# vLAR-group/OGC

Measured on AMD Instinct MI355X. Metric: point-clouds/sec (8192 pts) segnet fwd+bwd, higher is better.
Workload: dtype f32; 1 GPU; C4 KITTI-SF train_seg unsup: segnet_kitti fwd + OGC loss (dynamic+smooth+invariance) + bwd + Adam, 4 samples x 4 views x 8192 pts per GPU; n_point=8192, n_slot=10, parallelism=dp1, optimizer_stepped=True

## Files before the change

include/ogc_ops.h:

```cpp
#ifndef OGC_OPS_H
#define OGC_OPS_H

#ifdef __cplusplus
extern "C" {
#endif

typedef void *ogc_stream_t;
typedef unsigned short ogc_bf16_t;

enum {
    OGC_OK = 0,
    OGC_ERR_INVALID_ARG = -1,
    OGC_ERR_LAUNCH = -2,
    OGC_ERR_UNSUPPORTED = -3
};

#define OGC_VERSION 205
int ogc_version(void);
int ogc_distance_contracted(void);
int ogc_set_deterministic(int on);
int ogc_get_deterministic(void);
const char *ogc_last_error(void);

int ogc_furthest_point_sampling(int b, int n, int m, const float *xyz, float *temp,
                                int *idx, ogc_stream_t stream);

int ogc_furthest_point_sampling_chain(int b, int n, int m, const float *xyz, float *temp, int *idx,
                                      const int *ties_in, int *ties_out, ogc_stream_t stream);

int ogc_gather_points(int b, int c, int n, int npoints, const float *points, const int *idx,
                      float *out, ogc_stream_t stream);

int ogc_gather_points_grad(int b, int c, int n, int npoints, const float *grad_out,
                           const int *idx, float *grad_points, ogc_stream_t stream);

int ogc_knn(int b, int n, int m, int k, const float *unknown, const float *known,
            float *dist2, int *idx, ogc_stream_t stream);

int ogc_three_nn(int b, int n, int m, const float *unknown, const float *known, float *dist2,
                 int *idx, ogc_stream_t stream);

int ogc_three_interpolate(int b, int c, int m, int n, const float *points, const int *idx,
                          const float *weight, float *out, ogc_stream_t stream);

int ogc_three_interpolate_grad(int b, int c, int n, int m, const float *grad_out,
                               const int *idx, const float *weight, float *grad_points,
                               ogc_stream_t stream);

int ogc_group_points(int b, int c, int n, int npoints, int nsample, const float *points,
                     const int *idx, float *out, ogc_stream_t stream);

int ogc_group_points_grad(int b, int c, int n, int npoints, int nsample, const float *grad_out,
                          const int *idx, float *grad_points, ogc_stream_t stream);

int ogc_ball_query(int b, int n, int m, float radius, int nsample, const float *new_xyz,
                   const float *xyz, int *idx, ogc_stream_t stream);


int ogc_knn_clamped(int b, int n, int m, int k, float radius, const float *unknown,
                    const float *known, float *dist, int *idx, ogc_stream_t stream);

long long ogc_cell_grid_bytes(int b, int n);
int ogc_cell_grid_build(int b, int n, float radius, const float *xyz, void *grid, ogc_stream_t stream);
int ogc_ball_query_cells(int b, int n, float radius, int nsample, const float *xyz, const void *grid, float grid_radius, int *idx,
                         ogc_stream_t stream);
int ogc_knn_clamped_cells(int b, int n, int k, float radius, const float *xyz, void *grid, float grid_radius, float *dist, int *idx,
                          ogc_stream_t stream);

int ogc_adam_max_tensors(void);
int ogc_adam_chunk(void);
int ogc_adam_step(int n_tensors, int n_chunks, const long long *table, const int *chunks, const void *const *grad_ptrs,
                  float *step_snapshot, int *flag, double lr, double beta1, double beta2, double eps, double weight_decay,
                  ogc_stream_t stream);

int ogc_kabsch_rotation(int nb, const float *S, float *R, int *valid, ogc_stream_t stream);

int ogc_group_concat(int b, int c, int n, int npoints, int nsample, const float *xyz, const float *new_xyz,
                     const float *points, const int *idx, float *out, ogc_stream_t stream);

int ogc_group_concat_grad(int b, int c, int n, int npoints, int nsample, const float *grad_out, const int *idx,
                          float *grad_points, ogc_stream_t stream);

int ogc_group_linear_fwd(int b, int m, int n, int npoints, int nsample, int groups, const float *P, const int *idx,
                         const float *rel, const float *wx, float *y, double *stats, ogc_stream_t stream);
int ogc_group_linear_fwd_direct(int b, int m, int cf, int n, int npoints, int nsample, int groups, const float *feats,
                                const int *idx, const float *rel, const float *w, float *y, double *stats, ogc_stream_t stream);
int ogc_group_linear_fwd_direct_h(int b, int m, int cf, int n, int npoints, int nsample, int groups, const float *feats,
                                  const int *idx, const float *rel, const float *w, ogc_bf16_t *y, double *stats, ogc_stream_t stream);
int ogc_group_linear_bwd(int b, int m, int n, int npoints, int nsample, const float *grad_y, const int *idx,
                         const float *rel, float *grad_p, float *dwx, ogc_stream_t stream);

int ogc_group_reverse_chunk(int n, int npoints, int nsample);
int ogc_group_reverse(int b, int n, int npoints, int nsample, const int *idx, int *rev_start, unsigned short *rev_pos,
                      unsigned short *heads, ogc_stream_t stream);
int ogc_group_points_grad_rev(int b, int c, int n, int npoints, int nsample, const float *grad_out, const int *rev_start,
                              const unsigned short *rev_pos, const unsigned short *heads, float *grad_points,
                              ogc_stream_t stream);

int ogc_group_points_grad_rev_dwx(int b, int c, int n, int npoints, int nsample, const float *grad_out, const int *rev_start,
                                  const unsigned short *rev_pos, const unsigned short *heads, const float *rel,
// ... 73 lines not shown

int ogc_mlp_chain_pool_supported(int c0, int c1, int c2, int c3, int nsample);
int ogc_mlp_chain_pool(int b, int c0, int c1, int c2, int c3, int p, int nsample, const float *x, const float *wt1,
                       const float *b1, const float *wt2, const float *b2, const float *wt3, const float *b3, float *out,
                       ogc_stream_t stream);

int ogc_corr_layer_pool_supported(int cf, int c1, int c2, int c3, int nsample);
int ogc_corr_layer_pool(int b, int cf, int c1, int c2, int c3, int n1, int n2, int nsample, const float *pos1,
                        const float *pos2, const float *feat1, const float *feat2, const int *idx, const float *wt1,
                        const float *b1, const float *wt2, const float *b2, const float *wt3, const float *b3, float *out,
                        ogc_stream_t stream);

long long ogc_slot_masks_ws_floats(int b, int d, int n, int k);
int ogc_slot_masks_fwd(int b, int d, int n, int k, float temperature, const float *feats, const float *slots,
                       float *mask, ogc_stream_t stream);
int ogc_slot_masks_bwd(int b, int d, int n, int k, float temperature, const float *feats, const float *slots,
                       const float *mask, const float *grad_mask, float *grad_feats, float *grad_slots, float *ws,
                       ogc_stream_t stream);

int ogc_group_norm_stats_slots(void);
int ogc_group_norm_bwd_slots(void);
int ogc_group_norm_fwd(int b, int c, int hw, int groups, float eps, int relu, const float *x,
                       const float *gamma, const float *beta, float *y, float *mean, float *rstd,
                       double *ws, ogc_stream_t stream);
int ogc_group_norm_bwd(int b, int c, int hw, int groups, int relu, const float *x, const float *gamma,
                       const float *beta, const float *mean, const float *rstd, const float *grad_y,
                       float *grad_x, float *grad_gamma, float *grad_beta, double *ws, ogc_stream_t stream);

int ogc_group_norm_maxpool_fwd(int b, int c, int p, int s, int groups, float eps, int relu, const float *x,
                               const float *gamma, const float *beta, float *out, int *argmax, float *mean,
                               float *rstd, double *ws, ogc_stream_t stream);
int ogc_group_norm_maxpool_bwd(int b, int c, int p, int s, int groups, int relu, const float *x,
                               const float *gamma, const float *mean, const float *rstd, const float *out,
                               const int *argmax, const float *grad_out, float *grad_x, float *grad_gamma,
                               float *grad_beta, double *ws, ogc_stream_t stream);
int ogc_group_norm_maxpool_bwd_ext(int b, int c, int p, int s, int groups, int relu, const float *x,
                                   const float *x_at_argmax, const float *gamma, const float *mean, const float *rstd,
                                   const float *out, const int *argmax, const float *grad_out, float *grad_x,
                                   float *grad_gamma, float *grad_beta, double *ws, ogc_stream_t stream);

int ogc_batch_norm_fwd(int b, int c, int hw, float eps, int relu, int training, float momentum, const float *x,
                       const float *gamma, const float *beta, float *running_mean, float *running_var, float *y,
                       float *mean, float *rstd, double *ws, const double *stats, int slots, ogc_stream_t stream);
int ogc_batch_norm_bwd(int b, int c, int hw, int relu, int training, const float *x, const float *gamma,
                       const float *beta, const float *mean, const float *rstd, const float *grad_y, float *grad_x,
                       float *grad_gamma, float *grad_beta, double *ws, ogc_stream_t stream);
int ogc_batch_norm_maxpool_fwd(int b, int c, int p, int s, float eps, int relu, int training, float momentum,
                               const float *x, const float *gamma, const float *beta, float *running_mean,
                               float *running_var, float *out, int *argmax, float *mean, float *rstd, double *ws,
                               const double *stats, int slots, ogc_stream_t stream);
int ogc_batch_norm_maxpool_bwd(int b, int c, int p, int s, int relu, int training, const float *x, const float *gamma,
                               const float *mean, const float *rstd, const float *out, const int *argmax,
                               const float *grad_out, float *grad_x, float *grad_gamma, float *grad_beta, double *ws,
                               ogc_stream_t stream);

int ogc_conv1x1_wgrad(int b, int cin, int cout, int hw, const float *x, const float *dy, float *dw,
                      ogc_stream_t stream);

int ogc_conv1x1_gemm(int b, int M, int K, int hw, int transpose_a, const float *w, const float *in,
                     float *out, ogc_stream_t stream);

int ogc_conv1x1_gn_slots(void);
int ogc_conv1x1_gemm_stats_supported(int b, int M, int K, int hw, int affine);
int ogc_conv1x1_gemm_stream_supported(int b, int M, int K, int hw);
int ogc_conv1x1_gemm_any(int b, int M, int K, int hw, int transpose_a, const float *w, const float *in, float *out,
                         ogc_stream_t stream);

int ogc_set_matmul_precision(int bf16);
int ogc_conv1x1_gemm_gnstats(int b, int M, int K, int hw, int groups, const float *w, const float *in, float *out,
                             double *stats, ogc_stream_t stream);

int ogc_group_norm_coeffs(int b, int c, int hw, int groups, float eps, const float *x, const float *gamma,
                          const float *beta, const double *stats, int slots, double *ws, float *mean, float *rstd,
                          float *a, float *bb, ogc_stream_t stream);
int ogc_conv1x1_gemm_affine(int b, int M, int K, int hw, int relu, int groups, const float *w, const float *in,
                            const float *pa, const float *pb, float *out, double *stats, ogc_stream_t stream);
int ogc_conv1x1_wgrad_affine(int b, int cin, int cout, int hw, int relu, const float *x, const float *pa,
                             const float *pb, const float *dy, float *dw, ogc_stream_t stream);
int ogc_conv1x1_wgrad_affine_pooled(int b, int cin, int cout, int hw, int relu, int nsample, const float *x, const float *pa,
                                    const float *pb, const float *y, const float *coef2, const float *inj, float *dw,
                                    ogc_stream_t stream);
int ogc_conv1x1_dgrad_pooled(int b, int cin, int cout, int hw, int nsample, const float *w, const float *y, const float *coef2,
                             const float *inj, float *grad_z, ogc_stream_t stream);

int ogc_group_norm_fwd_stats(int b, int c, int hw, int groups, float eps, int relu, const float *x,
                             const float *gamma, const float *beta, float *y, float *mean, float *rstd,
                             const double *stats, int slots, ogc_stream_t stream);
int ogc_group_norm_maxpool_fwd_stats(int b, int c, int p, int s, int groups, float eps, int relu, const float *x,
                                     const float *gamma, const float *beta, float *out, int *argmax, float *mean,
                                     float *rstd, const double *stats, int slots, ogc_stream_t stream);

int ogc_conv1x1_gemm_affine_pool(int b, int M, int K, int hw, int relu, int groups, int nsample, const float *w,
                                 const float *in, const float *pa, const float *pb, const float *next_gamma,
                                 float *out, double *stats, float *yext, int *aext, ogc_stream_t stream);
int ogc_group_norm_pool_extremes(int b, int c, int p, int s, int groups, float eps, int relu, const float *yext,
                                 const int *aext, const float *gamma, const float *beta, float *out, int *argmax,
                                 float *mean, float *rstd, const double *stats, int slots, ogc_stream_t stream);

int ogc_chamfer_terms(int b, int n1, int n2, int p, const float *p1, const float *pc2, const int *idx12, const int *idx21,
                      float *dist1, float *dist2, ogc_stream_t stream);
int ogc_chamfer_terms_grad(int b, int n1, int n2, int p, const float *p1, const float *pc2, const int *idx12, const int *idx21,
                           const float *g1, const float *g2, float *grad_p1, ogc_stream_t stream);

int ogc_gather_xyz_pair(int b, int n, int m, const float *xyz, const int *idx, float *out, float *out_t, ogc_stream_t stream);
int ogc_flow_advance(int b, int n, float scale, const float *cur, const float *delta, const float *ref, float *out_delta,
                     float *out_new, float *out_new_t, float *out_flow, ogc_stream_t stream);
int ogc_linear_cn(int b, int cin, int cout, int n, const float *x, const float *weight, const float *bias, float *y,
                  ogc_stream_t stream);
int ogc_three_nn_weights(int b, int n, int mode, const float *dist2, float *weight, ogc_stream_t stream);
int ogc_soft_corr_flow(int b, int n1, int n2, int c, float support, const float *epsilon, const float *pc1, const float *pc2,
                       const float *f1, const float *f2, float *flow, ogc_stream_t stream);
int ogc_gru_reset(int b, int c, int cx, int n, int s, const float *rc, long long rc_batch_stride, const float *hx, float *out,
                  ogc_stream_t stream);
int ogc_gru_blend(int b, int c, int n, int s, const float *zc, long long zc_batch_stride, const float *qc,
                  long long qc_batch_stride, const float *h, long long h_batch_stride, float *out, ogc_stream_t stream);

int ogc_zero_arena_begin(void *base, int bytes, ogc_stream_t stream);
int ogc_zero_arena_end(void);

int ogc_group_linear_fwd_h(int b, int m, int n, int npoints, int nsample, int groups, const float *P, const int *idx,
                           const float *rel, const float *wx, ogc_bf16_t *y, double *stats, ogc_stream_t stream);
int ogc_group_linear_fwd_pt_h(int b, int m, int n, int npoints, int nsample, int groups, const float *Pt, const int *idx,
                              const float *rel, const float *wx, ogc_bf16_t *y, double *stats, ogc_stream_t stream);
int ogc_group_points_grad_rev_h(int b, int c, int n, int npoints, int nsample, const ogc_bf16_t *grad_out, const int *rev_start,
                                const unsigned short *rev_pos, const unsigned short *heads, float *grad_points,
                                ogc_stream_t stream);
int ogc_group_points_grad_rev_dwx_h(int b, int c, int n, int npoints, int nsample, const ogc_bf16_t *grad_out, const int *rev_start,
                                    const unsigned short *rev_pos, const unsigned short *heads, const float *rel,
                                    float *grad_points, float *dwx, ogc_stream_t stream);
int ogc_conv1x1_gemm_h(int b, int M, int K, int hw, int transpose_a, const float *w, const ogc_bf16_t *in, ogc_bf16_t *out,
                       ogc_stream_t stream);
int ogc_conv1x1_gemm_affine_h(int b, int M, int K, int hw, int relu, int groups, const float *w, const ogc_bf16_t *in,
                              const float *pa, const float *pb, ogc_bf16_t *out, double *stats, ogc_stream_t stream);
int ogc_conv1x1_gemm_affine_pool_h(int b, int M, int K, int hw, int relu, int groups, int nsample, const float *w,
                                   const ogc_bf16_t *in, const float *pa, const float *pb, const float *next_gamma,
                                   ogc_bf16_t *out, double *stats, float *yext, int *aext, ogc_stream_t stream);
int ogc_conv1x1_wgrad_xf_h(int b, int cin, int cout, int hw, const float *x, const ogc_bf16_t *dy, float *dw,
                           ogc_stream_t stream);
int ogc_conv1x1_wgrad_affine_h(int b, int cin, int cout, int hw, int relu, const ogc_bf16_t *x, const float *pa,
                               const float *pb, const ogc_bf16_t *dy, float *dw, ogc_stream_t stream);
int ogc_conv1x1_wgrad_affine_pooled_h(int b, int cin, int cout, int hw, int relu, int nsample, const ogc_bf16_t *x,
                                      const float *pa, const float *pb, const ogc_bf16_t *y, const float *coef2,
                                      const float *inj, float *dw, ogc_stream_t stream);
int ogc_conv1x1_dgrad_pooled_h(int b, int cin, int cout, int hw, int nsample, const float *w, const ogc_bf16_t *y,
                               const float *coef2, const float *inj, ogc_bf16_t *grad_z, ogc_stream_t stream);
int ogc_conv1x1_wgrad_moments_h(int b, int cin, int cout, int hw, int relu, const ogc_bf16_t *y_prev, const float *pa,
                                const float *pb, const ogc_bf16_t *grad_y, float *moments, ogc_stream_t stream);
int ogc_conv1x1_wgrad_moments_pooled_h(int b, int cin, int cout, int hw, int relu, int nsample, const ogc_bf16_t *y_prev,
                                       const float *pa, const float *pb, const ogc_bf16_t *y, const float *coef2,
                                       const float *inj, float *moments, ogc_stream_t stream);
int ogc_conv1x1_dgrad_adjoint_h(int b, int cin, int cout, int hw, int relu, const float *w, const ogc_bf16_t *grad_y,
                                const ogc_bf16_t *y_prev, const float *pa, const float *pb, const float *coef,
                                ogc_bf16_t *grad_prev, ogc_stream_t stream);
int ogc_conv1x1_dgrad_adjoint_pooled_h(int b, int cin, int cout, int hw, int relu, int nsample, const float *w,
                                       const ogc_bf16_t *y, const float *coef2, const float *inj, const ogc_bf16_t *y_prev,
                                       const float *pa, const float *pb, const float *coef, ogc_bf16_t *grad_prev,
                                       ogc_stream_t stream);
int ogc_group_norm_bwd_h(int b, int c, int hw, int groups, int relu, const ogc_bf16_t *x, const float *gamma,
                         const float *beta, const float *mean, const float *rstd, const ogc_bf16_t *grad_y,
                         ogc_bf16_t *grad_x, float *grad_gamma, float *grad_beta, double *ws, ogc_stream_t stream);
int ogc_group_norm_maxpool_bwd_sparse_h(int b, int c, int p, int s, int groups, int relu, const ogc_bf16_t *x,
                                        const float *x_at_argmax, const float *gamma, const float *mean, const float *rstd,
                                        const float *out, const int *argmax, const float *grad_out, float *coef2, float *inj,
                                        float *grad_gamma, float *grad_beta, double *ws, ogc_stream_t stream);

#ifdef __cplusplus
// ... 4 lines not shown
```

ogc_amd/_lib.py:

```python
import ctypes
import os

_HERE = os.path.dirname(os.path.abspath(__file__))
FMAD = os.environ.get("OGC_FMAD", "0") == "1"
DETERMINISTIC = os.environ.get("OGC_DETERMINISTIC", "0") == "1"
LIB_PATH = os.path.join(_HERE, "csrc", "libogc_ops_fmad.so" if FMAD else "libogc_ops.so")

_vp = ctypes.c_void_p
_int = ctypes.c_int
_flt = ctypes.c_float
_dbl = ctypes.c_double
_ll = ctypes.c_longlong

SIGNATURES = {
    "ogc_set_deterministic": [_int],
    "ogc_group_linear_fwd_direct": [_int, _int, _int, _int, _int, _int, _int, _vp, _vp, _vp, _vp, _vp, _vp, _vp],
    "ogc_get_deterministic": [],
    "ogc_furthest_point_sampling": [_int, _int, _int, _vp, _vp, _vp, _vp],
    "ogc_furthest_point_sampling_chain": [_int, _int, _int, _vp, _vp, _vp, _vp, _vp, _vp],
    "ogc_gather_points": [_int, _int, _int, _int, _vp, _vp, _vp, _vp],
    "ogc_gather_points_grad": [_int, _int, _int, _int, _vp, _vp, _vp, _vp],
    "ogc_knn": [_int, _int, _int, _int, _vp, _vp, _vp, _vp, _vp],
    "ogc_three_nn": [_int, _int, _int, _vp, _vp, _vp, _vp, _vp],
    "ogc_three_interpolate": [_int, _int, _int, _int, _vp, _vp, _vp, _vp, _vp],
# ... 7 lines not shown
    "ogc_view_means_grad": [_int, _vp, _vp, _vp, _vp, _vp, _vp],
    "ogc_sum_ranges": [_int, _vp, _vp, _vp, _ll, _vp, _vp],
    "ogc_three_interpolate_grad_rev_bs": [_int, _int, _int, _int, _vp, _ll, _vp, _vp, _vp, _vp, _vp, _vp],
    "ogc_group_points_grad_rev": [_int, _int, _int, _int, _int, _vp, _vp, _vp, _vp, _vp, _vp],
    "ogc_group_points_grad_rev_dwx": [_int, _int, _int, _int, _int, _vp, _vp, _vp, _vp, _vp, _vp, _vp, _vp],
    "ogc_ball_query": [_int, _int, _int, _flt, _int, _vp, _vp, _vp, _vp],
    "ogc_knn_clamped": [_int, _int, _int, _int, _flt, _vp, _vp, _vp, _vp, _vp],
    "ogc_cell_grid_bytes": [_int, _int],
    "ogc_cell_grid_build": [_int, _int, _flt, _vp, _vp, _vp],
    "ogc_ball_query_cells": [_int, _int, _flt, _int, _vp, _vp, _flt, _vp, _vp],
    "ogc_knn_clamped_cells": [_int, _int, _int, _flt, _vp, _vp, _flt, _vp, _vp, _vp],
    "ogc_chamfer_terms": [_int, _int, _int, _int, _vp, _vp, _vp, _vp, _vp, _vp, _vp],
    "ogc_chamfer_terms_grad": [_int, _int, _int, _int, _vp, _vp, _vp, _vp, _vp, _vp, _vp, _vp],
    "ogc_gather_xyz_pair": [_int, _int, _int, _vp, _vp, _vp, _vp, _vp],
    "ogc_flow_advance": [_int, _int, _flt, _vp, _vp, _vp, _vp, _vp, _vp, _vp, _vp],
    "ogc_linear_cn": [_int, _int, _int, _int, _vp, _vp, _vp, _vp, _vp],
    "ogc_three_nn_weights": [_int, _int, _int, _vp, _vp, _vp],
    "ogc_soft_corr_flow": [_int, _int, _int, _int, _flt, _vp, _vp, _vp, _vp, _vp, _vp, _vp],
    "ogc_gru_reset": [_int, _int, _int, _int, _int, _vp, _ll, _vp, _vp, _vp],
    "ogc_gru_blend": [_int, _int, _int, _int, _vp, _ll, _vp, _ll, _vp, _ll, _vp, _vp],
    "ogc_zero_arena_begin": [_vp, _int, _vp],
    "ogc_zero_arena_end": [],
    "ogc_adam_max_tensors": [],
    "ogc_adam_chunk": [],
    "ogc_adam_step": [_int, _int, _vp, _vp, _vp, _vp, _vp, _dbl, _dbl, _dbl, _dbl, _dbl, _vp],
    "ogc_kabsch_rotation": [_int, _vp, _vp, _vp, _vp],
    "ogc_lsap_maximize": [_int, _int, _vp, _vp, _vp],
    "ogc_rigid_moments": [_int, _int, _int, _vp, _vp, _vp, _vp, _vp, _vp, _vp],
    "ogc_rigid_translation": [_int, _vp, _vp, _vp, _vp, _vp],
    "ogc_rigid_blend": [_int, _int, _int, _int, _int, _vp, _vp, _vp, _vp, _vp, _vp, _vp, _vp],
    "ogc_mask_iou": [_int, _int, _int, _vp, _vp, _vp, _vp, _vp],
    "ogc_matched_distance": [_int, _int, _int, _int, _int, _vp, _vp, _vp, _vp, _vp, _vp, _vp, _vp, _vp],
    "ogc_soft_nn_target": [_int, _int, _int, _int, _flt, _vp, _vp, _vp, _vp, _vp, _vp],
    "ogc_group_concat": [_int, _int, _int, _int, _int, _vp, _vp, _vp, _vp, _vp, _vp],
    "ogc_group_linear_fwd": [_int, _int, _int, _int, _int, _int, _vp, _vp, _vp, _vp, _vp, _vp, _vp],
    "ogc_group_linear_bwd": [_int, _int, _int, _int, _int, _vp, _vp, _vp, _vp, _vp, _vp],
    "ogc_group_concat_grad": [_int, _int, _int, _int, _int, _vp, _vp, _vp, _vp],
    "ogc_neighbour_consistency_fwd": [_int, _int, _int, _int, _int, _vp, _vp, _vp, _vp],
    "ogc_reverse_neighbours": [_int, _int, _int, _vp, _vp, _vp, _vp, _vp, _vp],
    "ogc_neighbour_consistency_bwd": [_int, _int, _int, _int, _int, _vp, _vp, _vp, _vp, _vp, _vp, _vp, _vp],
    "ogc_sym_eigvals": [_int, _int, _vp, _vp, _vp],
    "ogc_group_norm_fwd": [_int, _int, _int, _int, _flt, _int, _vp, _vp, _vp, _vp, _vp, _vp, _vp, _vp],
    "ogc_group_norm_bwd": [_int, _int, _int, _int, _int, _vp, _vp, _vp, _vp, _vp, _vp, _vp, _vp, _vp, _vp, _vp],
    "ogc_group_norm_maxpool_fwd": [_int, _int, _int, _int, _int, _flt, _int, _vp, _vp, _vp, _vp, _vp, _vp, _vp, _vp, _vp],
    "ogc_conv1x1_gemm": [_int, _int, _int, _int, _int, _vp, _vp, _vp, _vp],
    "ogc_attention_fwd": [_int, _int, _int, _int, _int, _flt, _vp, _int, _vp, _int, _vp, _int, _vp, _vp, _vp],
    "ogc_attention_bwd": [_int, _int, _int, _int, _int, _flt, _vp, _int, _vp, _int, _vp, _int, _vp, _vp, _vp, _vp, _int,
                          _vp, _int, _vp, _int, _vp],
    "ogc_conv1x1_gemm_affine_pool": [_int, _int, _int, _int, _int, _int, _int, _vp, _vp, _vp, _vp, _vp, _vp, _vp, _vp, _vp,
                                     _vp],
    "ogc_group_norm_pool_extremes": [_int, _int, _int, _int, _int, _flt, _int, _vp, _vp, _vp, _vp, _vp, _vp, _vp, _vp, _vp,
                                     _int, _vp],
    "ogc_small_linear_fwd": [_int, _int, _int, _vp, _vp, _vp, _vp, _vp],
    "ogc_small_linear_bwd": [_int, _int, _int, _vp, _vp, _vp, _vp, _vp, _vp, _vp],
    "ogc_conv1x1_wgrad_moments": [_int, _int, _int, _int, _int, _vp, _vp, _vp, _vp, _vp, _vp],
    "ogc_gn_moments_combine": [_int, _int, _int, _int, _int, _vp, _vp, _vp, _vp, _vp, _vp, _vp, _vp, _vp, _vp, _vp, _vp],
    "ogc_conv1x1_dgrad_adjoint": [_int, _int, _int, _int, _int, _vp, _vp, _vp, _vp, _vp, _vp, _vp, _vp],
    "ogc_group_norm_maxpool_bwd_sparse": [_int, _int, _int, _int, _int, _int, _vp, _vp, _vp, _vp, _vp, _vp, _vp, _vp, _vp, _vp,
                                          _vp, _vp, _vp, _vp],
    "ogc_group_norm_maxpool_bwd_ext": [_int, _int, _int, _int, _int, _int, _vp, _vp, _vp, _vp, _vp, _vp, _vp, _vp, _vp, _vp,
                                       _vp, _vp, _vp],
    "ogc_conv1x1_wgrad_moments_pooled": [_int, _int, _int, _int, _int, _int, _vp, _vp, _vp, _vp, _vp, _vp, _vp, _vp],
    "ogc_conv1x1_dgrad_adjoint_pooled": [_int, _int, _int, _int, _int, _int, _vp, _vp, _vp, _vp, _vp, _vp, _vp, _vp, _vp, _vp],
    "ogc_mlp_chain_pool_supported": [_int, _int, _int, _int, _int],
    "ogc_mlp_chain_pool": [_int, _int, _int, _int, _int, _int, _int, _vp, _vp, _vp, _vp, _vp, _vp, _vp, _vp, _vp],
    "ogc_corr_layer_pool_supported": [_int, _int, _int, _int, _int],
    "ogc_corr_layer_pool": [_int, _int, _int, _int, _int, _int, _int, _int, _vp, _vp, _vp, _vp, _vp, _vp, _vp, _vp, _vp, _vp,
                            _vp, _vp, _vp],
    "ogc_slot_masks_ws_floats": [_int, _int, _int, _int],
    "ogc_slot_masks_fwd": [_int, _int, _int, _int, _flt, _vp, _vp, _vp, _vp],
    "ogc_slot_masks_bwd": [_int, _int, _int, _int, _flt, _vp, _vp, _vp, _vp, _vp, _vp, _vp, _vp],
    "ogc_conv1x1_gn_slots": [],
    "ogc_conv1x1_gemm_stats_supported": [_int, _int, _int, _int, _int],
    "ogc_conv1x1_gemm_stream_supported": [_int, _int, _int, _int],
    "ogc_conv1x1_gemm_any": [_int, _int, _int, _int, _int, _vp, _vp, _vp, _vp],
    "ogc_set_matmul_precision": [_int],
    "ogc_group_norm_stats_slots": [],
    "ogc_group_norm_bwd_slots": [],
    "ogc_group_norm_coeffs": [_int, _int, _int, _int, _flt, _vp, _vp, _vp, _vp, _int, _vp, _vp, _vp, _vp, _vp, _vp],
    "ogc_conv1x1_gemm_affine": [_int, _int, _int, _int, _int, _int, _vp, _vp, _vp, _vp, _vp, _vp, _vp],
    "ogc_conv1x1_wgrad_affine": [_int, _int, _int, _int, _int, _vp, _vp, _vp, _vp, _vp, _vp],
    "ogc_conv1x1_wgrad_affine_pooled": [_int, _int, _int, _int, _int, _int, _vp, _vp, _vp, _vp, _vp, _vp, _vp, _vp],
    "ogc_conv1x1_dgrad_pooled": [_int, _int, _int, _int, _int, _vp, _vp, _vp, _vp, _vp, _vp],
    "ogc_batch_norm_fwd": [_int, _int, _int, _flt, _int, _int, _flt, _vp, _vp, _vp, _vp, _vp, _vp, _vp, _vp, _vp, _vp,
                           _int, _vp],
    "ogc_batch_norm_bwd": [_int, _int, _int, _int, _int, _vp, _vp, _vp, _vp, _vp, _vp, _vp, _vp, _vp, _vp, _vp],
    "ogc_batch_norm_maxpool_fwd": [_int, _int, _int, _int, _flt, _int, _int, _flt, _vp, _vp, _vp, _vp, _vp, _vp, _vp,
                                   _vp, _vp, _vp, _vp, _int, _vp],
    "ogc_batch_norm_maxpool_bwd": [_int, _int, _int, _int, _int, _int, _vp, _vp, _vp, _vp, _vp, _vp, _vp, _vp, _vp,
                                   _vp, _vp, _vp],
    "ogc_conv1x1_gemm_gnstats": [_int, _int, _int, _int, _int, _vp, _vp, _vp, _vp, _vp],
    "ogc_group_norm_fwd_stats": [_int, _int, _int, _int, _flt, _int, _vp, _vp, _vp, _vp, _vp, _vp, _vp, _int, _vp],
    "ogc_group_norm_maxpool_fwd_stats": [_int, _int, _int, _int, _int, _flt, _int, _vp, _vp, _vp, _vp, _vp, _vp, _vp,
                                         _vp, _int, _vp],
    "ogc_conv1x1_wgrad": [_int, _int, _int, _int, _vp, _vp, _vp, _vp],
    "ogc_group_norm_maxpool_bwd": [_int, _int, _int, _int, _int, _int, _vp, _vp, _vp, _vp, _vp, _vp, _vp, _vp, _vp, _vp,
                                   _vp, _vp],
}

for _n in ("ogc_group_linear_fwd", "ogc_group_points_grad_rev", "ogc_conv1x1_gemm", "ogc_conv1x1_gemm_affine",
           "ogc_conv1x1_gemm_affine_pool", "ogc_conv1x1_wgrad_affine", "ogc_conv1x1_wgrad_affine_pooled",
           "ogc_conv1x1_dgrad_pooled", "ogc_conv1x1_wgrad_moments", "ogc_conv1x1_wgrad_moments_pooled",
           "ogc_conv1x1_dgrad_adjoint", "ogc_conv1x1_dgrad_adjoint_pooled", "ogc_group_norm_bwd",
           "ogc_group_norm_maxpool_bwd_sparse", "ogc_group_points_grad_rev_dwx"):
    SIGNATURES[_n + "_h"] = SIGNATURES[_n]
SIGNATURES["ogc_group_linear_fwd_direct_h"] = SIGNATURES["ogc_group_linear_fwd_direct"]
SIGNATURES["ogc_conv1x1_wgrad_xf_h"] = SIGNATURES["ogc_conv1x1_wgrad"]
SIGNATURES["ogc_group_linear_fwd_pt_h"] = SIGNATURES["ogc_group_linear_fwd"]

HEADER_VERSION = 205
_lib = None
_fns = {}


class OgcOpsError(RuntimeError):
    pass


def load():
    global _lib
    if _lib is None:
        if not os.path.exists(LIB_PATH):
            raise OgcOpsError(
                "libogc_ops.so not found at %s — build it with `python ogc_amd/csrc/build.py` "
                "(there is no CPU fallback)" % LIB_PATH)
        L = ctypes.CDLL(LIB_PATH)
        for name, argtypes in SIGNATURES.items():
            fn = getattr(L, name)
            fn.argtypes = argtypes
            fn.restype = _int
        L.ogc_version.restype = _int
        if L.ogc_version() != HEADER_VERSION:
            raise OgcOpsError("libogc_ops.so at %s is version %d, this package binds version %d of include/ogc_ops.h — rebuild it "
                              "with `python ogc_amd/csrc/build.py --force`" % (LIB_PATH, L.ogc_version(), HEADER_VERSION))
        L.ogc_distance_contracted.restype = _int
        if bool(L.ogc_distance_contracted()) != FMAD:
            raise OgcOpsError("%s evaluates distances %s, OGC_FMAD asked for the other form" %
                              (LIB_PATH, "contracted (fma)" if L.ogc_distance_contracted() else "un-contracted"))
        L.ogc_slot_masks_ws_floats.restype = ctypes.c_longlong
        L.ogc_cell_grid_bytes.restype = ctypes.c_longlong
        L.ogc_last_error.restype = ctypes.c_char_p
        L.ogc_set_deterministic(1 if DETERMINISTIC else 0)
        _lib = L
    return _lib


def set_deterministic(on):
    global DETERMINISTIC
    DETERMINISTIC = bool(on)
    load().ogc_set_deterministic(1 if on else 0)


CALL_COUNTS = None

ROCTX_NAMES = {
    "ogc_furthest_point_sampling": "K1 furthest_point_sampling", "ogc_furthest_point_sampling_chain": "K1 furthest_point_sampling (chain)",
    "ogc_gather_points": "K2 gather_points", "ogc_gather_points_grad": "K3 gather_points_grad",
    "ogc_knn": "K4 knn", "ogc_knn_clamped": "K4 knn (+ sqrt + radius clamp)", "ogc_knn_clamped_cells": "K4 knn (shared cell grid)",
    "ogc_three_nn": "K5 three_nn", "ogc_three_interpolate": "K6 three_interpolate",
    "ogc_three_interpolate_grad": "K7 three_interpolate_grad", "ogc_three_interpolate_grad_rev": "K7 three_interpolate_grad (gather form)",
    "ogc_three_interpolate_grad_rev_bs": "K7 three_interpolate_grad (gather form)",
    "ogc_group_points": "K8 group_points", "ogc_group_points_grad": "K9 group_points_grad",
    "ogc_group_points_grad_rev": "K9 group_points_grad (gather form)",
    "ogc_ball_query": "K10 ball_query", "ogc_ball_query_cells": "K10 ball_query (shared cell grid)",
}
_roctx = None


def _roctx_lib():
    global _roctx
    if _roctx is None:
        _roctx = False
        if os.environ.get("OGC_ROCTX", "0") == "1":
            for name in ("librocprofiler-sdk-roctx.so", "libroctx64.so"):
                try:
                    lib = ctypes.CDLL(os.path.join(os.environ.get("ROCM_PATH", "/opt/rocm"), "lib", name))
                    lib.roctxRangePushA.argtypes = [ctypes.c_char_p]
                    lib.roctxRangePushA.restype = ctypes.c_int
                    lib.roctxRangePop.restype = ctypes.c_int
                    _roctx = lib
                    break
                except (OSError, AttributeError):
                    continue
    return _roctx


def call(name, *args):
    if CALL_COUNTS is not None:
        CALL_COUNTS[name] += 1
    fn = _fns.get(name)
    if fn is None:
        fn = _fns[name] = getattr(load(), name)
    tx = _roctx_lib()
# ... 13 lines not shown
```

ogc_amd/csrc/conv1x1.hip:

```cpp
#include "conv1x1_shared.h"
#include "act_io.h"
#include "conv1x1_epilogue.h"

int ogc_g_matmul_bf16 = 0;


namespace {


template <bool TRANSPOSE_A, int KQ, bool STATS, bool PRO, bool BF, bool POOL = false, typename IT = float, typename OT = float>
__global__ __launch_bounds__(WG_WAVES *OGC_WAVE) void conv1x1_gemm_kernel(int M, int K, int hw, int groups,
                                                                          const float *__restrict__ w,
                                                                          const IT *__restrict__ in,
                                                                          OT *__restrict__ out,
                                                                          double *__restrict__ stats,
                                                                          const float *__restrict__ pa,
                                                                          const float *__restrict__ pb, int pro_relu,
                                                                          PoolOut pool = PoolOut()) {
    extern __shared__ __attribute__((aligned(16))) float a_lds[];
    __shared__ double s_stats[STATS ? 64 : 1];
    __shared__ __attribute__((aligned(16))) float s_sign[POOL ? 64 : 4];
    const int lane = threadIdx.x & 63, wave = threadIdx.x >> 6;
    const int j = lane & 15, kk = lane >> 4;
    const int b = blockIdx.y;
// ... 132 lines not shown
#pragma unroll
        for (int q = 0; q < KQ; ++q) {
            if (q < Kq) {
                float av[4];
#pragma unroll
                for (int a = 0; a < 4; ++a) av[a] = a_lds[(a * 16 + j) * a_ld + q * 4 + kk];
#pragma unroll
                for (int a = 0; a < 4; ++a) {
                    if (a < nblk) {
                        acc[a][0] = __builtin_amdgcn_mfma_f32_16x16x4f32(av[a], xin[q].x, acc[a][0], 0, 0, 0);
                        acc[a][1] = __builtin_amdgcn_mfma_f32_16x16x4f32(av[a], xin[q].y, acc[a][1], 0, 0, 0);
                        acc[a][2] = __builtin_amdgcn_mfma_f32_16x16x4f32(av[a], xin[q].z, acc[a][2], 0, 0, 0);
                        acc[a][3] = __builtin_amdgcn_mfma_f32_16x16x4f32(av[a], xin[q].w, acc[a][3], 0, 0, 0);
                    }
                }
            }
        }
        }
        if (live) {
            if constexpr (sizeof(OT) == 2 && (STATS || POOL)) {
#pragma unroll
                for (int a = 0; a < 4; ++a)
#pragma unroll
                    for (int c = 0; c < 4; ++c)
#pragma unroll
                        for (int r = 0; r < 4; ++r) acc[a][c][r] = ogc_as_stored<OT>(acc[a][c][r]);
            }
#pragma unroll
            for (int a = 0; a < 4; ++a)
#pragma unroll
                for (int r = 0; r < 4; ++r) {
                    const int m = m0 + a * 16 + kk * 4 + r;
                    if (m < M) {
                        const float4 o = make_float4(acc[a][0][r], acc[a][1][r], acc[a][2][r], acc[a][3][r]);
                        ogc_st4(outb + (size_t)m * hw + p0 + 4 * j, o);
                    }
                }
            if constexpr (POOL) {
                const int centres = hw / pool.s;
                const int centre = (p0 + 4 * j) / pool.s;
                const size_t o0 = ((size_t)b * M + m0 + kk * 4) * centres + centre;
                if (pool.s == 64) ogc_pool_extremes_epilogue<16>(acc, nblk, s_sign, j, kk, m0, M, centres, 64, pool.yext + o0, pool.aext + o0);
                else if (pool.s == 32) ogc_pool_extremes_epilogue<8>(acc, nblk, s_sign, j, kk, m0, M, centres, 32, pool.yext + o0, pool.aext + o0);
                else ogc_pool_extremes_epilogue<4>(acc, nblk, s_sign, j, kk, m0, M, centres, 16, pool.yext + o0, pool.aext + o0);
            }
            if (STATS) {
#pragma unroll
                for (int a = 0; a < 4; ++a) {
                    if (a < nblk) {
                        float sm = 0.f, sq = 0.f;
#pragma unroll
                        for (int r = 0; r < 4; ++r)
#pragma unroll
                            for (int c = 0; c < 4; ++c) {
                                const float v = acc[a][c][r];
                                sm += v;
                                sq += v * v;
                            }
                        sm += ogc_dpp_f32<0xB1>(sm); sq += ogc_dpp_f32<0xB1>(sq);
                        sm += ogc_dpp_f32<0x4E>(sm); sq += ogc_dpp_f32<0x4E>(sq);
                        sm += ogc_dpp_f32<0x141>(sm); sq += ogc_dpp_f32<0x141>(sq);
                        sm += ogc_dpp_f32<0x140>(sm); sq += ogc_dpp_f32<0x140>(sq);
                        const int m = m0 + a * 16 + kk * 4;
                        if (j == 0 && m < M) {
                            const int g = m / cpg;
                            atomicAdd(&s_stats[2 * g], (double)sm);
                            atomicAdd(&s_stats[2 * g + 1], (double)sq);
                        }
                    }
                }
            }
        }
    }
    if (STATS) {
        __syncthreads();
        if (threadIdx.x < 2 * groups) {
            const int slot = blockIdx.x % GN_SLOTS;
            double *dst = stats + ((size_t)slot * gridDim.y + b) * 2 * groups;
            atomicAdd(dst + threadIdx.x, s_stats[threadIdx.x]);
        }
    }
}

template <int KQ, bool PRO, bool EXACT, bool STATS = false, bool POOL = false, bool DUAL = false, bool TRANS = false>
__global__ __launch_bounds__(WG_WAVES *OGC_WAVE, DUAL ? 2 : 1) void conv1x1_gemm_stream_kernel(int M, int K, int hw, int ntiles,
                                                                                 const float *__restrict__ w,
                                                                                 const float *__restrict__ in,
                                                                                 float *__restrict__ out,
                                                                                 const float *__restrict__ pa,
                                                                                 const float *__restrict__ pb, int pro_relu,
                                                                                 int groups = 1, int nbatch = 1,
                                                                                 double *__restrict__ stats = nullptr,
                                                                                 PoolOut pool = PoolOut()) {
    extern __shared__ __attribute__((aligned(16))) float a_lds[];
    const int lane = threadIdx.x & 63, wave = __builtin_amdgcn_readfirstlane(threadIdx.x >> 6);
    const int j = lane & 15, kk = lane >> 4;
    const int Kq = (K + 3) >> 2, Mt = (M + 63) >> 6, a_ld = ogc_a_ld(Kq);
    const int tiles_per_img = hw >> 6;
    for (int mt = 0; mt < Mt; ++mt)
        ogc_stage_weight_tile<TRANS, WG_WAVES>(a_lds + (size_t)mt * 64 * a_ld, w, mt * 64, M, K, Kq);
    float *sgn_all = a_lds + (size_t)Mt * 64 * a_ld + (PRO ? WG_WAVES * 2 * FW_KQ_MAX * 4 : 0) + WG_WAVES * 4 * 16 * 2 * 2;
    if constexpr (POOL) {
        for (int t = threadIdx.x; t < Mt * 64; t += WG_WAVES * OGC_WAVE) sgn_all[t] = (t < M && pool.sign[t] < 0.f) ? -1.f : 1.f;
    }
    __syncthreads();
    const int nw = gridDim.x * WG_WAVES;
    const unsigned off_main = (unsigned)(kk * hw + 4 * j);
    const unsigned off_last = (unsigned)(min(kk, K - 1 - (Kq - 1) * 4) * hw + 4 * j);
    auto load_tile = [&](int t, float4(&x)[KQ]) {
        t = min(t, ntiles - 1);
        const int b = t / tiles_per_img, p0 = (t - b * tiles_per_img) * 64;
        const float *inb = in + (size_t)b * K * hw + p0;
#pragma unroll
        for (int q = 0; q < KQ; ++q)
            if (EXACT || q < Kq) {
                const float *rowq = inb + (size_t)(q * 4) * hw;
                x[q] = *reinterpret_cast<const float4 *>(rowq + ((EXACT ? q == KQ - 1 : q == Kq - 1) ? off_last : off_main));
            }
    };
    float *cw = a_lds + (size_t)Mt * 64 * a_ld + wave * (2 * KQ * 4);
    int coef_b = -1;
    double *sacc = reinterpret_cast<double *>(a_lds + (size_t)Mt * 64 * a_ld + (PRO ? WG_WAVES * 2 * FW_KQ_MAX * 4 : 0)) +
                   wave * (4 * 16 * 2);
    int stat_b = -1;
    auto flush_stats = [&]() {
        if constexpr (STATS) {
            if (stat_b >= 0) {
                const int cpg = M / groups;
                double *dst = stats + ((size_t)(blockIdx.x % GN_SLOTS) * nbatch + stat_b) * 2 * groups;
                if (lane < Mt * 16) {
                    const int m = (lane >> 4) * 64 + ((lane >> 2) & 3) * 16 + (lane & 3) * 4;
                    if (m < M) {
                        unsafeAtomicAdd(dst + 2 * (m / cpg), sacc[2 * lane]);
                        unsafeAtomicAdd(dst + 2 * (m / cpg) + 1, sacc[2 * lane + 1]);
                    }
                }
            }
            if (lane < 64) { sacc[2 * lane] = 0.0; sacc[2 * lane + 1] = 0.0; }
            __builtin_amdgcn_wave_barrier();
        }
    };
    auto compute_store = [&](int t, float4(&x)[KQ]) {
        const int b = t / tiles_per_img, p0 = (t - b * tiles_per_img) * 64;
        if constexpr (STATS) {
            if (b != stat_b) { flush_stats(); stat_b = b; }
        }
        if (PRO) {
            if (b != coef_b) {
                coef_b = b;
                for (int r = lane; r < KQ * 4; r += OGC_WAVE) {
                    cw[r] = r < K ? pa[(size_t)b * K + r] : 0.f;
                    cw[KQ * 4 + r] = r < K ? pb[(size_t)b * K + r] : 0.f;
                }
                __builtin_amdgcn_wave_barrier();
            }
#pragma unroll
            for (int q = 0; q < KQ; ++q) {
                if (EXACT || q < Kq) {
                    const float ca = cw[q * 4 + kk], cb = cw[KQ * 4 + q * 4 + kk];
                    float4 v = x[q];
                    v.x = fmaf(ca, v.x, cb); v.y = fmaf(ca, v.y, cb);
                    v.z = fmaf(ca, v.z, cb); v.w = fmaf(ca, v.w, cb);
                    if (pro_relu) { v.x = fmaxf(v.x, 0.f); v.y = fmaxf(v.y, 0.f); v.z = fmaxf(v.z, 0.f); v.w = fmaxf(v.w, 0.f); }
                    x[q] = v;
                }
            }
        }
        float *outb = out + (size_t)b * M * hw + p0;
        const unsigned off_out = (unsigned)(kk * 4 * hw + 4 * j);
        for (int mt = 0; mt < Mt; ++mt) {
            const float *at = a_lds + (size_t)mt * 64 * a_ld;
            const int nblk = EXACT ? 4 : min(4, (M - mt * 64 + 15) >> 4);
            v4f acc[4][4];
#pragma unroll
            for (int a = 0; a < 4; ++a)
#pragma unroll
                for (int c = 0; c < 4; ++c) acc[a][c] = (v4f){0.f, 0.f, 0.f, 0.f};
#pragma unroll
            for (int q = 0; q < KQ; ++q) {
                if (EXACT || q < Kq) {
                    float av[4];
#pragma unroll
                    for (int a = 0; a < 4; ++a) av[a] = at[(a * 16 + j) * a_ld + q * 4 + kk];
#pragma unroll
                    for (int a = 0; a < 4; ++a) {
                        if (EXACT || a < nblk) {
                            acc[a][0] = __builtin_amdgcn_mfma_f32_16x16x4f32(av[a], x[q].x, acc[a][0], 0, 0, 0);
                            acc[a][1] = __builtin_amdgcn_mfma_f32_16x16x4f32(av[a], x[q].y, acc[a][1], 0, 0, 0);
                            acc[a][2] = __builtin_amdgcn_mfma_f32_16x16x4f32(av[a], x[q].z, acc[a][2], 0, 0, 0);
                            acc[a][3] = __builtin_amdgcn_mfma_f32_16x16x4f32(av[a], x[q].w, acc[a][3], 0, 0, 0);
                        }
                    }
                }
            }
#pragma unroll
            for (int a = 0; a < 4; ++a)
#pragma unroll
                for (int r = 0; r < 4; ++r) {
                    const int m0 = mt * 64 + a * 16 + r;
                    if (EXACT || m0 + kk * 4 < M)
                        *reinterpret_cast<float4 *>(outb + (size_t)m0 * hw + off_out) =
                            make_float4(acc[a][0][r], acc[a][1][r], acc[a][2][r], acc[a][3][r]);
                }
            if constexpr (POOL) {
                const int m0p = mt * 64;
                const int centres = hw / pool.s;
                const int centre = (p0 + 4 * j) / pool.s;
                const size_t o0 = ((size_t)b * M + m0p + kk * 4) * centres + centre;
                const float *sg = sgn_all + m0p;
                if (pool.s == 64) ogc_pool_extremes_epilogue<16>(acc, nblk, sg, j, kk, m0p, M, centres, 64, pool.yext + o0, pool.aext + o0);
                else if (pool.s == 32) ogc_pool_extremes_epilogue<8>(acc, nblk, sg, j, kk, m0p, M, centres, 32, pool.yext + o0, pool.aext + o0);
                else ogc_pool_extremes_epilogue<4>(acc, nblk, sg, j, kk, m0p, M, centres, 16, pool.yext + o0, pool.aext + o0);
            }
            if constexpr (STATS) {
#pragma unroll
                for (int a = 0; a < 4; ++a) {
                    if (EXACT || a < nblk) {
                        float sm = 0.f, sq = 0.f;
#pragma unroll
                        for (int r = 0; r < 4; ++r)
#pragma unroll
                            for (int c = 0; c < 4; ++c) {
                                const float v = acc[a][c][r];
                                sm += v;
                                sq += v * v;
                            }
                        sm += ogc_dpp_f32<0xB1>(sm); sq += ogc_dpp_f32<0xB1>(sq);
                        sm += ogc_dpp_f32<0x4E>(sm); sq += ogc_dpp_f32<0x4E>(sq);
                        sm += ogc_dpp_f32<0x141>(sm); sq += ogc_dpp_f32<0x141>(sq);
                        sm += ogc_dpp_f32<0x140>(sm); sq += ogc_dpp_f32<0x140>(sq);
                        if (j == 0) {
                            const int slot = (mt * 4 + a) * 4 + kk;
                            sacc[2 * slot] += (double)sm;
                            sacc[2 * slot + 1] += (double)sq;
                        }
                    }
                }
            }
        }
    };
    const int per = (ntiles + nw - 1) / nw;
    int t = (blockIdx.x * WG_WAVES + wave) * per;
    const int t_end = min(ntiles, t + per);
    if (STATS) flush_stats();
    if constexpr (DUAL) {
        float4 x1[KQ];
        for (; t < t_end; ++t) {
            load_tile(t, x1);
            compute_store(t, x1);
        }
        if (STATS) flush_stats();
        return;
    }
    float4 xa[KQ], xb[KQ];
    if (t < t_end) {
        load_tile(t, xa);
        for (; t + 1 < t_end; t += 2) {
            load_tile(t + 1, xb);
            compute_store(t, xa);
            load_tile(t + 2, xa);
            compute_store(t + 1, xb);
        }
        if (t < t_end) compute_store(t, xa);
    }
    if (STATS) flush_stats();
}

bool gemm_stream_eligible(int b, int M, int K, int hw, bool pro, bool pool = false, bool any_precision = false) {
    const int Kq = (K + 3) / 4, Mt = (M + 63) / 64;
    const long long ntiles = (long long)b * (hw / 64);
    const size_t lds = ((size_t)Mt * 64 * ogc_a_ld(Kq) + (pro ? WG_WAVES * 2 * FW_KQ_MAX * 4 : 0)) * sizeof(float) +
                       WG_WAVES * 4 * 16 * 2 * sizeof(double) + (pool ? (size_t)Mt * 64 * sizeof(float) : 0);
    static const bool off = getenv("OGC_GEMM_STREAM") && getenv("OGC_GEMM_STREAM")[0] == '0';
    return !(off || (g_matmul_bf16 && !any_precision) || (hw & 63) != 0 || Kq <= 25 || Kq > FW_KQ_MAX || lds > 156 * 1024 || ntiles < 2048 ||
             ntiles >= (1ll << 31));
}

template <bool PRO, bool STATS = false, bool POOL = false, bool TRANS = false>
bool gemm_stream_launch(int b, int M, int K, int hw, const float *w, const float *in, float *out, const float *pa,
                        const float *pb, int pro_relu, hipStream_t s, int groups = 1, double *stats = nullptr,
                        PoolOut pool = PoolOut()) {
    const int Kq = (K + 3) / 4, Mt = (M + 63) / 64;
    const long long ntiles = (long long)b * (hw / 64);
    const size_t lds = ((size_t)Mt * 64 * ogc_a_ld(Kq) + (PRO ? WG_WAVES * 2 * FW_KQ_MAX * 4 : 0)) * sizeof(float) +
                       WG_WAVES * 4 * 16 * 2 * sizeof(double) + (POOL ? (size_t)Mt * 64 * sizeof(float) : 0);
    if (!gemm_stream_eligible(b, M, K, hw, PRO, POOL, STATS) || lds > 156 * 1024) return false;
    const int wgs = (int)(ntiles / WG_WAVES < 256 ? ntiles / WG_WAVES : 256);
#define OGC_STREAM_D(KQV, EX, DU, WGS)                                                                                       \
    do {                                                                                                                     \
        static bool raised = false;                                                                                          \
        const void *fn = reinterpret_cast<const void *>(&conv1x1_gemm_stream_kernel<KQV, PRO, EX, STATS, POOL, DU, TRANS>);         \
        if (!raised) {                                                                                                       \
            if (hipFuncSetAttribute(fn, hipFuncAttributeMaxDynamicSharedMemorySize, 156 * 1024) != hipSuccess) return false;  \
            raised = true;                                                                                                   \
        }                                                                                                                    \
        hipLaunchKernelGGL((conv1x1_gemm_stream_kernel<KQV, PRO, EX, STATS, POOL, DU, TRANS>), dim3(WGS), dim3(WG_WAVES * OGC_WAVE), \
                           lds, s, M, K, hw, (int)ntiles, w, in, out, pa, pb, pro_relu, groups, b, stats, pool);             \
    } while (0)
    static const bool dual_on = !(getenv("OGC_GEMM_STREAM_DUAL") && getenv("OGC_GEMM_STREAM_DUAL")[0] == '0');
    const bool dual = dual_on && !POOL && 2 * (lds + 1024) <= 156 * 1024 && ntiles >= 4096;
    const int wgs2 = (int)(ntiles / WG_WAVES < 512 ? ntiles / WG_WAVES : 512);
#define OGC_STREAM(KQV, EX)                                                                                                  \
    do {                                                                                                                     \
        if (dual) OGC_STREAM_D(KQV, EX, true, wgs2);                                                                         \
        else OGC_STREAM_D(KQV, EX, false, wgs);                                                                              \
    } while (0)
    const bool full_rows = M % 64 == 0;
    if (Kq == 32 && full_rows) OGC_STREAM(32, true);
    else if (Kq == 33 && full_rows) OGC_STREAM(33, true);
    else if (Kq <= 33) OGC_STREAM(33, false);
    else OGC_STREAM(40, false);
#undef OGC_STREAM
#undef OGC_STREAM_D
    return true;
}

template <bool T, bool STATS, bool PRO, bool POOL = false, typename AT = float>
int gemm_launch(int b, int M, int K, int hw, int groups, const float *w, const AT *in, AT *out, double *stats,
                const float *pa, const float *pb, int pro_relu, hipStream_t s, PoolOut pool = PoolOut()) {
    const int Kq = (K + 3) / 4;
    constexpr bool F32 = sizeof(AT) == 4;
    if constexpr (F32 && !T && (!POOL || (STATS && PRO))) {
        static const bool wide_fp32 = [] { const char *e = getenv("OGC_BF16_WIDE_STATS"); return e && e[0] == '1'; }();
        if ((!g_matmul_bf16 || (STATS && wide_fp32)) &&
            gemm_stream_launch<PRO, STATS, POOL>(b, M, K, hw, w, in, out, pa, pb, pro_relu, s, groups, stats, pool))
            return OGC_OK;
    }
    if constexpr (F32 && T && !STATS && !PRO && !POOL) {
        if (!g_matmul_bf16 && gemm_stream_launch<false, false, false, true>(b, M, K, hw, w, in, out, pa, pb, pro_relu, s))
            return OGC_OK;
    }
    if constexpr (F32) {
        if (!g_matmul_bf16 && ogc_gemm32_launch(T, STATS, PRO, POOL, b, M, K, hw, groups, w, in, out, stats, pa, pb, pro_relu, s,
                                                pool.sign, pool.yext, pool.aext, pool.s))
            return OGC_OK;
    }
    if constexpr (!F32) {
        if (ogc_gemm16_launch(T, STATS, PRO, POOL, b, M, K, hw, groups, w, in, out, stats, pa, pb, pro_relu, s, pool.sign, pool.yext,
                              pool.aext, pool.s))
            return OGC_OK;
    }
    const size_t lds = (size_t)64 * ogc_a_ld(Kq) * sizeof(float);
    dim3 grid(ogc_divup(hw, 64 * WG_WAVES), b);
#define OGC_GEMM(KQV)                                                                                                  \
    do {                                                                                                               \
        if constexpr (!F32)                                                                                            \
            hipLaunchKernelGGL((conv1x1_gemm_kernel<T, KQV, STATS, PRO, true, POOL, AT, AT>), grid,                     \
                               dim3(WG_WAVES * OGC_WAVE), lds, s, M, K, hw, groups, w, in, out, stats, pa, pb, pro_relu, pool); \
        else if (g_matmul_bf16)                                                                                        \
            hipLaunchKernelGGL((conv1x1_gemm_kernel<T, KQV, STATS, PRO, true, POOL>), grid, dim3(WG_WAVES * OGC_WAVE), \
                               lds, s, M, K, hw, groups, w, in, out, stats, pa, pb, pro_relu, pool);                   \
        else                                                                                                           \
            hipLaunchKernelGGL((conv1x1_gemm_kernel<T, KQV, STATS, PRO, false, POOL>), grid, dim3(WG_WAVES * OGC_WAVE), \
                               lds, s, M, K, hw, groups, w, in, out, stats, pa, pb, pro_relu, pool);                   \
    } while (0)
    if (Kq <= 2) OGC_GEMM(2);
    else if (Kq <= 8) OGC_GEMM(8);
    else if (Kq <= 16) OGC_GEMM(16);
    else if (Kq <= 25) OGC_GEMM(25);
    else if (POOL && !g_matmul_bf16) return OGC_ERR_UNSUPPORTED;
    else {
        if (Kq <= 33) OGC_GEMM(33);
        else OGC_GEMM(40);
    }
#undef OGC_GEMM
    return OGC_OK;
}

template <typename AT>
int gemm_check(const char *name, int b, int M, int K, int hw, const float *w, const AT *in, const AT *out) {
    OGC_REQUIRE(b >= 0 && M >= 1 && K >= 1 && hw >= 1, "%s: bad shape", name);
    OGC_REQUIRE(w && in && out, "%s: null pointer", name);
    if ((hw & 63) != 0 || K > 4 * FW_KQ_MAX || (((uintptr_t)in | (uintptr_t)out) & ogc_act_mask<AT>()) != 0) {
        ogc_set_error("%s: needs hw %% 64 == 0, K <= %d and 16-byte aligned tensors (hw=%d, K=%d)", name,
                      4 * FW_KQ_MAX, hw, K);
        return OGC_ERR_UNSUPPORTED;
    }
    if (sizeof(AT) == 2 && !g_matmul_bf16) {
        ogc_set_error("%s: 16-bit activations need ogc_set_matmul_precision(1)", name);
        return OGC_ERR_UNSUPPORTED;
    }
    OGC_REQUIRE((long long)M * hw < (1ll << 31) && (long long)K * hw < (1ll << 31) && b <= 65535,
                "%s: one sample exceeds 32-bit indexing", name);
    return OGC_OK;
}

}

namespace {
template <typename AT>
int gemm_plain_impl(const char *name, int b, int M, int K, int hw, int transpose_a, const float *w, const AT *in, AT *out,
                    ogc_stream_t stream) {
    const int rc = gemm_check(name, b, M, K, hw, w, in, out);
    if (rc != OGC_OK) return rc;
    if (b == 0) return OGC_OK;
    if (transpose_a)
        gemm_launch<true, false, false, false, AT>(b, M, K, hw, 1, w, in, out, nullptr, nullptr, nullptr, 0, (hipStream_t)stream);
    else
        gemm_launch<false, false, false, false, AT>(b, M, K, hw, 1, w, in, out, nullptr, nullptr, nullptr, 0, (hipStream_t)stream);
    OGC_CHECK_LAUNCH(name);
    return OGC_OK;
}
}

extern "C" int ogc_conv1x1_gemm(int b, int M, int K, int hw, int transpose_a, const float *w, const float *in,
                                float *out, ogc_stream_t stream) {
    return gemm_plain_impl<float>("ogc_conv1x1_gemm", b, M, K, hw, transpose_a, w, in, out, stream);
}

extern "C" int ogc_conv1x1_gemm_h(int b, int M, int K, int hw, int transpose_a, const float *w, const ogc_bf16_t *in,
                                  ogc_bf16_t *out, ogc_stream_t stream) {
    return gemm_plain_impl<ogc_bf16>("ogc_conv1x1_gemm_h", b, M, K, hw, transpose_a, w, in, out, stream);
}

extern "C" int ogc_conv1x1_gn_slots(void) { return GN_SLOTS; }

extern "C" int ogc_conv1x1_gemm_stats_supported(int b, int M, int K, int hw, int affine) {
    if (b < 1 || M < 1 || K < 1 || hw < 1) return 0;
    return (K <= 100 || g_matmul_bf16 || gemm_stream_eligible(b, M, K, hw, affine != 0, false, true)) ? 1 : 0;
}

extern "C" int ogc_conv1x1_gemm_stream_supported(int b, int M, int K, int hw) {
    if (b < 1 || M < 1 || K < 1 || hw < 1) return 0;
    return gemm_stream_eligible(b, M, K, hw, false) ? 1 : 0;
}

extern "C" int ogc_set_matmul_precision(int bf16) {
    const int previous = g_matmul_bf16;
    g_matmul_bf16 = bf16 ? 1 : 0;
    return previous;
}

extern "C" int ogc_conv1x1_gemm_gnstats(int b, int M, int K, int hw, int groups, const float *w, const float *in,
                                        float *out, double *stats, ogc_stream_t stream) {
    const int rc = gemm_check<float>("ogc_conv1x1_gemm_gnstats", b, M, K, hw, w, in, out);
    if (rc != OGC_OK) return rc;
    OGC_REQUIRE(stats, "ogc_conv1x1_gemm_gnstats: null pointer");
    if (groups < 1 || groups > 32 || M % groups != 0 || (M / groups) % 4 != 0) {
        ogc_set_error("ogc_conv1x1_gemm_gnstats: needs 1 <= groups <= 32 and (M / groups) %% 4 == 0 (M=%d, groups=%d)", M,
                      groups);
        return OGC_ERR_UNSUPPORTED;
    }
    if (K > 100 && !g_matmul_bf16 && !gemm_stream_eligible(b, M, K, hw, false, false, true)) {
        ogc_set_error("ogc_conv1x1_gemm_gnstats: not profitable for K > 100 (K=%d) on this shape; use ogc_conv1x1_gemm", K);
        return OGC_ERR_UNSUPPORTED;
    }
    if (b == 0) return OGC_OK;
    if (ogc_zero_async(stats, sizeof(double) * 2 * GN_SLOTS * (size_t)b * groups, (hipStream_t)stream) != hipSuccess) {
        ogc_set_error("ogc_conv1x1_gemm_gnstats: memset failed");
        return OGC_ERR_LAUNCH;
    }
    gemm_launch<false, true, false>(b, M, K, hw, groups, w, in, out, stats, nullptr, nullptr, 0, (hipStream_t)stream);
    OGC_CHECK_LAUNCH("ogc_conv1x1_gemm_gnstats");
    return OGC_OK;
}


namespace {
template <typename AT>
int gemm_affine_impl(const char *name, int b, int M, int K, int hw, int relu, int groups, const float *w, const AT *in,
                     const float *pa, const float *pb, AT *out, double *stats, ogc_stream_t stream) {
    const int rc = gemm_check(name, b, M, K, hw, w, in, out);
    if (rc != OGC_OK) return rc;
    OGC_REQUIRE(pa && pb, "ogc_conv1x1_gemm_affine: null pointer");
    if (b == 0) return OGC_OK;
    hipStream_t s = (hipStream_t)stream;
    if (groups > 0) {
        OGC_REQUIRE(stats, "ogc_conv1x1_gemm_affine: null pointer");
        if (groups > 32 || M % groups != 0 || (M / groups) % 4 != 0 || (K > 100 && !g_matmul_bf16 && !gemm_stream_eligible(b, M, K, hw, true, false, true))) {
            ogc_set_error("ogc_conv1x1_gemm_affine: output statistics need groups <= 32, (M / groups) %% 4 == 0, K <= 100 "
                          "(or a shape of the streaming kernel: ogc_conv1x1_gemm_stats_supported)");
            return OGC_ERR_UNSUPPORTED;
        }
        if (ogc_zero_async(stats, sizeof(double) * 2 * GN_SLOTS * (size_t)b * groups, s) != hipSuccess) {
            ogc_set_error("ogc_conv1x1_gemm_affine: memset failed");
            return OGC_ERR_LAUNCH;
        }
        gemm_launch<false, true, true, false, AT>(b, M, K, hw, groups, w, in, out, stats, pa, pb, relu, s);
    } else {
        gemm_launch<false, false, true, false, AT>(b, M, K, hw, 1, w, in, out, nullptr, pa, pb, relu, s);
    }
    OGC_CHECK_LAUNCH(name);
    return OGC_OK;
}
}

extern "C" int ogc_conv1x1_gemm_affine(int b, int M, int K, int hw, int relu, int groups, const float *w, const float *in,
                                       const float *pa, const float *pb, float *out, double *stats,
                                       ogc_stream_t stream) {
    return gemm_affine_impl<float>("ogc_conv1x1_gemm_affine", b, M, K, hw, relu, groups, w, in, pa, pb, out, stats, stream);
}

extern "C" int ogc_conv1x1_gemm_affine_h(int b, int M, int K, int hw, int relu, int groups, const float *w, const ogc_bf16_t *in,
                                         const float *pa, const float *pb, ogc_bf16_t *out, double *stats,
                                         ogc_stream_t stream) {
    return gemm_affine_impl<ogc_bf16>("ogc_conv1x1_gemm_affine_h", b, M, K, hw, relu, groups, w, in, pa, pb, out, stats, stream);
}

namespace {
template <typename AT>
int gemm_affine_pool_impl(const char *name, int b, int M, int K, int hw, int relu, int groups, int nsample, const float *w,
                          const AT *in, const float *pa, const float *pb, const float *next_gamma, AT *out, double *stats,
                          float *yext, int *aext, ogc_stream_t stream) {
    const int rc = gemm_check(name, b, M, K, hw, w, in, out);
// ... 40 lines not shown
```

ogc_amd/csrc/conv1x1_shared.h:

```cpp
#pragma once
#include <stdlib.h>

#include "ogc_common.h"
#include "conv_stage.h"

typedef float v4f __attribute__((ext_vector_type(4)));
typedef short v4s __attribute__((ext_vector_type(4)));

constexpr int WG_WAVES = 4;

extern int ogc_g_matmul_bf16;
#define g_matmul_bf16 ogc_g_matmul_bf16

__device__ __forceinline__ v4s ogc_pack_bf16(float a, float b, float c, float d) {
    typedef float v2f __attribute__((ext_vector_type(2)));
    typedef __bf16 v2bf __attribute__((ext_vector_type(2)));
    union { v2bf h[2]; v4s s; } u;
    u.h[0] = __builtin_convertvector((v2f){a, b}, v2bf);
    u.h[1] = __builtin_convertvector((v2f){c, d}, v2bf);
    return u.s;
}
```

ogc_amd/csrc/gemm_chunk.hip:

```cpp
#include <stdlib.h>

#include "ogc_common.h"
#include "act_io.h"
#include "conv1x1_shared.h"

namespace {

constexpr int GC_WAVES = 4;

__device__ __forceinline__ v4s gc_pack_bf16(float a, float b, float c, float d) { return ogc_pack_bf16_rr(a, b, c, d); }

template <int RB, int KQ, bool SPLIT_M, bool TRANS, bool POOLED = false, int KA = 1, typename AT = float, bool BF = false,
          bool TAB = false>
__global__ __launch_bounds__(GC_WAVES *OGC_WAVE, 2) void gemm_chunk_kernel(int M, int K, int hw, const float *__restrict__ w,
                                                                         const AT *__restrict__ in,
                                                                         AT *__restrict__ out,
                                                                         const float2 *__restrict__ coef2 = nullptr,
                                                                         const float2 *__restrict__ inj = nullptr,
                                                                         int s_shift = 0) {
    constexpr int KC = 4 * KQ, KCA = KC * KA, LD = 4 * ((KQ * KA) | 1);
    constexpr int MT = SPLIT_M ? 64 * RB : 16 * RB;
    constexpr int PER = (MT * KCA) / (GC_WAVES * OGC_WAVE);
    static_assert((MT * KCA) % (GC_WAVES * OGC_WAVE) == 0 && PER >= 1 && (KA == 1 || KA == 2), "staging split");
    extern __shared__ __attribute__((aligned(16))) float gc_lds[];
    const int t = threadIdx.x, lane = t & 63, wave = __builtin_amdgcn_readfirstlane(t >> 6);
    const int j = lane & 15, kk = lane >> 4;
    const int b = blockIdx.z;
    const int m0 = blockIdx.y * MT;
    const int wrow = SPLIT_M ? wave * 16 * RB : 0;
    const int p0 = SPLIT_M ? blockIdx.x * 64 : (blockIdx.x * GC_WAVES + wave) * 64;
    const bool active = p0 < hw;
    const int pl = active ? p0 : 0;
    const int nblk = min(RB, (M - m0 - wrow + 15) >> 4);
    const AT *inb = in + (size_t)b * K * hw + pl + 4 * j;
    const int nchunks = (K + KC - 1) / KC;

    v4f acc[RB][4];
#pragma unroll
    for (int a = 0; a < RB; ++a)
#pragma unroll
        for (int c = 0; c < 4; ++c) acc[a][c] = (v4f){0.f, 0.f, 0.f, 0.f};

    auto load_a = [&](int k0, float(&av)[PER]) {
#pragma unroll
        for (int i = 0; i < PER; ++i) {
            const int e = t + i * (GC_WAVES * OGC_WAVE);
            int mi, ki;
            if (TRANS) { mi = e % MT; ki = e / MT; } else { mi = e / KCA; ki = e % KCA; }
            const int m = m0 + mi, k = k0 + ki;
            const bool ok = m < M && k < K;
            const int mc = min(m, M - 1), kc = min(k, K - 1);
            const float v = TRANS ? w[(size_t)kc * M + mc] : w[(size_t)mc * K + kc];
            av[i] = ok ? v : 0.f;
        }
    };
    auto store_a = [&](float *dst, const float(&av)[PER]) {
#pragma unroll
        for (int i = 0; i < PER; ++i) {
            const int e = t + i * (GC_WAVES * OGC_WAVE);
            int mi, ki;
            if (TRANS) { mi = e % MT; ki = e / MT; } else { mi = e / KCA; ki = e % KCA; }
            dst[mi * LD + ki] = av[i];
        }
    };
    constexpr int NP = (POOLED && !TAB) ? KQ : 1;
    const int centres = hw >> s_shift;
    const int my_centre = (pl + 4 * j) >> s_shift, jpos = (pl + 4 * j) & ((1 << s_shift) - 1);
    const int cpw = 64 >> s_shift;
    float4 *tab = reinterpret_cast<float4 *>(gc_lds + 2 * MT * LD) + (size_t)wave * K * cpw;
    if constexpr (POOLED && TAB) {
        for (int e = lane; e < K * cpw; e += OGC_WAVE) {
            const int row = e / cpw, centre = (pl >> s_shift) + (e - row * cpw);
            const float2 c2v = coef2[(size_t)b * K + row];
            const float2 jj = centre < centres ? inj[((size_t)b * K + row) * centres + centre] : make_float2(0.f, __int_as_float(-1));
            tab[e] = make_float4(c2v.x, c2v.y, jj.x, jj.y);
        }
        __builtin_amdgcn_wave_barrier();
    }
    const int mine_c = (4 * j) >> s_shift;
    auto load_in = [&](int k0, float4(&xv)[KQ], float2(&cc)[NP], float2(&jv)[NP]) {
#pragma unroll
        for (int q = 0; q < KQ; ++q) {
            const int k = min(k0 + 4 * q + kk, K - 1);
            xv[q] = ogc_ld4(inb + (size_t)k * hw);
            if constexpr (POOLED && !TAB) {
                cc[q] = coef2[(size_t)b * K + k];
                jv[q] = inj[((size_t)b * K + k) * centres + my_centre];
            }
        }
    };
    auto rebuild = [&](int k0, float4(&xv)[KQ], const float2(&cc)[NP], const float2(&jv)[NP]) {
        if constexpr (POOLED && TAB) {
#pragma unroll
            for (int q = 0; q < KQ; ++q) {
                const float4 te = tab[min(k0 + 4 * q + kk, K - 1) * cpw + mine_c];
                const int rel = __float_as_int(te.w) - jpos;
                xv[q].x = fmaf(te.x, xv[q].x, te.y) + (rel == 0 ? te.z : 0.f);
                xv[q].y = fmaf(te.x, xv[q].y, te.y) + (rel == 1 ? te.z : 0.f);
                xv[q].z = fmaf(te.x, xv[q].z, te.y) + (rel == 2 ? te.z : 0.f);
                xv[q].w = fmaf(te.x, xv[q].w, te.y) + (rel == 3 ? te.z : 0.f);
            }
        } else if constexpr (POOLED) {
#pragma unroll
            for (int q = 0; q < KQ; ++q) {
                const int rel = __float_as_int(jv[q].y) - jpos;
                const float ag = jv[q].x;
                xv[q].x = fmaf(cc[q].x, xv[q].x, cc[q].y) + (rel == 0 ? ag : 0.f);
                xv[q].y = fmaf(cc[q].x, xv[q].y, cc[q].y) + (rel == 1 ? ag : 0.f);
                xv[q].z = fmaf(cc[q].x, xv[q].z, cc[q].y) + (rel == 2 ? ag : 0.f);
                xv[q].w = fmaf(cc[q].x, xv[q].w, cc[q].y) + (rel == 3 ? ag : 0.f);
            }
        }
        if (k0 + KC > K) {
#pragma unroll
            for (int q = 0; q < KQ; ++q)
                if (k0 + 4 * q + kk >= K) xv[q] = make_float4(0.f, 0.f, 0.f, 0.f);
        }
    };
    auto compute = [&](const float *a_lds, const float4(&xv)[KQ], int koff = 0) {
        if constexpr (BF) {
            static_assert(!BF || KQ % 4 == 0, "bf16 operands: whole groups of four row quads per input chunk");
#pragma unroll
            for (int g = 0; g < KQ / 4; ++g) {
                const float4 v0 = xv[4 * g], v1 = xv[4 * g + 1], v2 = xv[4 * g + 2], v3 = xv[4 * g + 3];
                const v4s bx = gc_pack_bf16(v0.x, v1.x, v2.x, v3.x);
                const v4s by = gc_pack_bf16(v0.y, v1.y, v2.y, v3.y);
                const v4s bz = gc_pack_bf16(v0.z, v1.z, v2.z, v3.z);
                const v4s bw = gc_pack_bf16(v0.w, v1.w, v2.w, v3.w);
                const float *ar = a_lds + (wrow + j) * LD + koff + 16 * g + kk;
#pragma unroll
                for (int a = 0; a < RB; ++a) {
                    const v4s av = gc_pack_bf16(ar[a * 16 * LD], ar[a * 16 * LD + 4], ar[a * 16 * LD + 8], ar[a * 16 * LD + 12]);
                    acc[a][0] = __builtin_amdgcn_mfma_f32_16x16x16bf16_1k(av, bx, acc[a][0], 0, 0, 0);
                    acc[a][1] = __builtin_amdgcn_mfma_f32_16x16x16bf16_1k(av, by, acc[a][1], 0, 0, 0);
                    acc[a][2] = __builtin_amdgcn_mfma_f32_16x16x16bf16_1k(av, bz, acc[a][2], 0, 0, 0);
                    acc[a][3] = __builtin_amdgcn_mfma_f32_16x16x16bf16_1k(av, bw, acc[a][3], 0, 0, 0);
                }
            }
        } else {
#pragma unroll
            for (int q = 0; q < KQ; ++q) {
                const float bx = xv[q].x, by = xv[q].y, bz = xv[q].z, bw = xv[q].w;
#pragma unroll
                for (int a = 0; a < RB; ++a) {
                    const float av = a_lds[(wrow + a * 16 + j) * LD + koff + q * 4 + kk];
                    acc[a][0] = __builtin_amdgcn_mfma_f32_16x16x4f32(av, bx, acc[a][0], 0, 0, 0);
                    acc[a][1] = __builtin_amdgcn_mfma_f32_16x16x4f32(av, by, acc[a][1], 0, 0, 0);
                    acc[a][2] = __builtin_amdgcn_mfma_f32_16x16x4f32(av, bz, acc[a][2], 0, 0, 0);
                    acc[a][3] = __builtin_amdgcn_mfma_f32_16x16x4f32(av, bw, acc[a][3], 0, 0, 0);
                }
            }
        }
    };

    float *buf0 = gc_lds, *buf1 = gc_lds + MT * LD;
    float4 x0[KQ], x1[KQ];
    float2 c0[NP], c1[NP], j0[NP], j1[NP];
    float a_next[PER];
    load_a(0, a_next);
    load_in(0, x0, c0, j0);
    store_a(buf0, a_next);
    __syncthreads();
    const bool work = nblk > 0;
    if constexpr (KA == 2) {
        const int npairs = (nchunks + 1) / 2;
        for (int p = 0; p < npairs; ++p) {
            const bool more = p + 1 < npairs;
            if (more) load_a((p + 1) * KCA, a_next);
            load_in((2 * p + 1) * KC, x1, c1, j1);
            rebuild(2 * p * KC, x0, c0, j0);
            if (work) compute(buf0, x0, 0);
            if (more) load_in((2 * p + 2) * KC, x0, c0, j0);
            rebuild((2 * p + 1) * KC, x1, c1, j1);
            if (work) compute(buf0, x1, KC);
            if (more) store_a(buf1, a_next);
            __syncthreads();
            float *tmp = buf0; buf0 = buf1; buf1 = tmp;
        }
    } else
    for (int i = 0; i < nchunks; i += 2) {
        const bool more1 = i + 1 < nchunks, more2 = i + 2 < nchunks;
        if (more1) {
            load_a((i + 1) * KC, a_next);
            load_in((i + 1) * KC, x1, c1, j1);
        }
        rebuild(i * KC, x0, c0, j0);
        if (work) compute(buf0, x0);
        if (more1) store_a(buf1, a_next);
        __syncthreads();
        if (!more1) break;
        if (more2) {
            load_a((i + 2) * KC, a_next);
            load_in((i + 2) * KC, x0, c0, j0);
        }
        rebuild((i + 1) * KC, x1, c1, j1);
        if (work) compute(buf1, x1);
        if (more2) store_a(buf0, a_next);
        __syncthreads();
    }
    if (!active) return;
    AT *ob = out + (size_t)b * M * hw + p0 + 4 * j;
#pragma unroll
    for (int a = 0; a < RB; ++a) {
        if (a < nblk) {
#pragma unroll
            for (int r = 0; r < 4; ++r) {
                const int m = m0 + wrow + a * 16 + kk * 4 + r;
                if (m < M) ogc_st4(ob + (size_t)m * hw, make_float4(acc[a][0][r], acc[a][1][r], acc[a][2][r], acc[a][3][r]));
            }
        }
    }
}

template <int RB, int KQ, bool SPLIT_M, int KA = 1>
void gemm_chunk_launch(int b, int M, int K, int hw, int transpose_a, const float *w, const float *in, float *out,
                       hipStream_t s) {
    constexpr int MT = SPLIT_M ? 64 * RB : 16 * RB;
    const size_t lds = (size_t)2 * MT * 4 * ((KQ * KA) | 1) * sizeof(float);
    dim3 grid(SPLIT_M ? hw / 64 : ogc_divup(hw, 64 * GC_WAVES), ogc_divup(M, MT), b);
#define GC_GO(TR, BFV)                                                                                                           \
    hipLaunchKernelGGL((gemm_chunk_kernel<RB, KQ, SPLIT_M, TR, false, KA, float, BFV>), grid, dim3(GC_WAVES * OGC_WAVE), lds, s, M, K, \
                       hw, w, in, out, nullptr, nullptr, 0)
    if (ogc_g_matmul_bf16) {
        if (transpose_a) GC_GO(true, true);
        else GC_GO(false, true);
    } else {
        if (transpose_a) GC_GO(true, false);
        else GC_GO(false, false);
    }
#undef GC_GO
}

}

extern "C" int ogc_conv1x1_gemm_any(int b, int M, int K, int hw, int transpose_a, const float *w, const float *in, float *out,
                                    ogc_stream_t stream) {
    OGC_REQUIRE(b >= 0 && M >= 1 && K >= 1 && hw >= 1, "ogc_conv1x1_gemm_any: bad shape");
    OGC_REQUIRE(w && in && out, "ogc_conv1x1_gemm_any: null pointer");
    if ((hw & 63) != 0 || (((uintptr_t)in | (uintptr_t)out) & 15) != 0) {
        ogc_set_error("ogc_conv1x1_gemm_any: needs hw %% 64 == 0 and 16-byte aligned tensors (hw=%d)", hw);
        return OGC_ERR_UNSUPPORTED;
    }
    OGC_REQUIRE((long long)M * hw < (1ll << 31) && (long long)K * hw < (1ll << 31) && b <= 65535,
                "ogc_conv1x1_gemm_any: one sample exceeds 32-bit indexing");
    if (b == 0) return OGC_OK;
    hipStream_t s = (hipStream_t)stream;
    const long long tiles = (long long)b * (hw / 64);
#define GC_CASE(RBV, KQV, SPLIT)                                                              \
    case RBV: gemm_chunk_launch<RBV, KQV, SPLIT>(b, M, K, hw, transpose_a, w, in, out, s); break
    if (tiles >= 4096) {
        const int ntile = ogc_divup(M, 128), rb = ogc_divup(M, 16 * ntile);
        switch (rb) {
            GC_CASE(1, 8, false); GC_CASE(2, 8, false); GC_CASE(3, 8, false); GC_CASE(4, 8, false);
            GC_CASE(5, 8, false); GC_CASE(6, 8, false); GC_CASE(7, 4, false);
            default: {
                static const char *kq = getenv("OGC_GEMM_CHUNK_KQ");
                if (kq && kq[0] == '4') gemm_chunk_launch<8, 4, false>(b, M, K, hw, transpose_a, w, in, out, s);
                else gemm_chunk_launch<8, 4, false, 2>(b, M, K, hw, transpose_a, w, in, out, s);
            }
        }
    } else {
        const bool same_rows = 128 * ogc_divup(M, 128) == 64 * ogc_divup(M, 64);
        const int rb = (M > 64 && same_rows && tiles * ogc_divup(M, 128) >= 512) ? 2 : 1;
        switch (rb) {
            GC_CASE(2, 8, true);
            default: gemm_chunk_launch<1, 8, true>(b, M, K, hw, transpose_a, w, in, out, s);
        }
    }
#undef GC_CASE
    OGC_CHECK_LAUNCH("ogc_conv1x1_gemm_any");
    return OGC_OK;
}

namespace {
template <typename AT>
int dgrad_pooled_impl(int b, int cin, int cout, int hw, int nsample, const float *w, const AT *y, const float *coef2,
                      const float *inj, AT *grad_z, ogc_stream_t stream) {
    constexpr bool BF = sizeof(AT) == 2;
    OGC_REQUIRE(b >= 0 && cin >= 1 && cout >= 1 && hw >= 1, "ogc_conv1x1_dgrad_pooled: bad shape");
    OGC_REQUIRE(w && y && coef2 && inj && grad_z, "ogc_conv1x1_dgrad_pooled: null pointer");
    const int sh = nsample == 16 ? 4 : nsample == 32 ? 5 : nsample == 64 ? 6 : -1;
    if (sh < 0 || hw % nsample != 0 || (hw & 63) != 0 || (long long)b * (hw / 64) < 1024 ||
        (((uintptr_t)y | (uintptr_t)grad_z) & ogc_act_mask<AT>()) != 0 || (((uintptr_t)coef2 | (uintptr_t)inj) & 7) != 0 ||
        (BF && !ogc_g_matmul_bf16)) {
        ogc_set_error("ogc_conv1x1_dgrad_pooled: needs nsample in {16, 32, 64} dividing hw, hw %% 64 == 0, >= 1024 tiles of 64 "
                      "positions and aligned tensors (hw=%d, nsample=%d, b=%d)", hw, nsample, b);
        return OGC_ERR_UNSUPPORTED;
    }
    OGC_REQUIRE((long long)cin * hw < (1ll << 31) && (long long)cout * hw < (1ll << 31) && b <= 65535,
                "ogc_conv1x1_dgrad_pooled: one sample exceeds 32-bit indexing");
    if (b == 0) return OGC_OK;
    hipStream_t s = (hipStream_t)stream;
    const float2 *c2 = reinterpret_cast<const float2 *>(coef2), *ij = reinterpret_cast<const float2 *>(inj);
    const int M = cin, K = cout;
    static const bool tab_off = [] { const char *e = getenv("OGC_DGRAD_POOLED_TAB"); return e && e[0] == '0'; }();
    const size_t tab_bytes = (size_t)GC_WAVES * K * (64 >> sh) * sizeof(float4);
    const bool tab = !tab_off && tab_bytes <= 24 * 1024;
    if (M <= 64) {
        constexpr int RB = 4, KQ = 4, KA = 2;
        dim3 grid(ogc_divup(hw, 64 * GC_WAVES), ogc_divup(M, 16 * RB), b);
        const size_t lds = (size_t)2 * 16 * RB * 4 * ((KQ * KA) | 1) * sizeof(float);
        if (tab)
            hipLaunchKernelGGL((gemm_chunk_kernel<RB, KQ, false, true, true, KA, AT, BF, true>), grid, dim3(GC_WAVES * OGC_WAVE),
                               lds + tab_bytes, s, M, K, hw, w, y, grad_z, c2, ij, sh);
        else
            hipLaunchKernelGGL((gemm_chunk_kernel<RB, KQ, false, true, true, KA, AT, BF>), grid, dim3(GC_WAVES * OGC_WAVE), lds, s, M,
                               K, hw, w, y, grad_z, c2, ij, sh);
    } else {
        constexpr int RB = 8, KQ = 4;
        dim3 grid(ogc_divup(hw, 64 * GC_WAVES), ogc_divup(M, 16 * RB), b);
        const size_t lds = (size_t)2 * 16 * RB * 4 * (KQ | 1) * sizeof(float);
        if (tab)
            hipLaunchKernelGGL((gemm_chunk_kernel<RB, KQ, false, true, true, 1, AT, BF, true>), grid, dim3(GC_WAVES * OGC_WAVE),
                               lds + tab_bytes, s, M, K, hw, w, y, grad_z, c2, ij, sh);
        else
            hipLaunchKernelGGL((gemm_chunk_kernel<RB, KQ, false, true, true, 1, AT, BF>), grid, dim3(GC_WAVES * OGC_WAVE), lds, s, M, K,
                               hw, w, y, grad_z, c2, ij, sh);
    }
    OGC_CHECK_LAUNCH("ogc_conv1x1_dgrad_pooled");
    return OGC_OK;
}
}

extern "C" int ogc_conv1x1_dgrad_pooled(int b, int cin, int cout, int hw, int nsample, const float *w, const float *y,
                                        const float *coef2, const float *inj, float *grad_z, ogc_stream_t stream) {
    return dgrad_pooled_impl<float>(b, cin, cout, hw, nsample, w, y, coef2, inj, grad_z, stream);
}

extern "C" int ogc_conv1x1_dgrad_pooled_h(int b, int cin, int cout, int hw, int nsample, const float *w, const ogc_bf16_t *y,
                                          const float *coef2, const float *inj, ogc_bf16_t *grad_z, ogc_stream_t stream) {
    return dgrad_pooled_impl<ogc_bf16>(b, cin, cout, hw, nsample, w, y, coef2, inj, grad_z, stream);
}
```

ogc_amd/csrc/group_norm.hip:

```cpp
#include "ogc_common.h"
#include "act_io.h"

namespace {

constexpr int GN_THREADS = 256;

__device__ __forceinline__ void gn_block_sum2(double &a, double &b, double *smem ) {
#pragma unroll
    for (int off = 32; off > 0; off >>= 1) {
        a += __shfl_down(a, off, 64);
        b += __shfl_down(b, off, 64);
    }
    const int lane = threadIdx.x & 63, wave = threadIdx.x >> 6;
    if (lane == 0) {
        smem[wave * 2] = a;
        smem[wave * 2 + 1] = b;
    }
    __syncthreads();
    if (threadIdx.x == 0) {
        a = 0.0;
        b = 0.0;
        for (int w = 0; w < GN_THREADS / 64; ++w) {
            a += smem[w * 2];
            b += smem[w * 2 + 1];
// ... 490 lines not shown
    const float a = rstd * gamma[ch];
    a_out[t] = a;
    bb_out[t] = beta[ch] - mean * a;
}
}

extern "C" int ogc_group_norm_coeffs(int b, int c, int hw, int groups, float eps, const float *x, const float *gamma,
                                     const float *beta, const double *stats, int slots, double *ws, float *mean,
                                     float *rstd, float *a, float *bb, ogc_stream_t stream) {
    OGC_REQUIRE(b >= 0 && c >= 1 && hw >= 1 && groups >= 1 && c % groups == 0, "ogc_group_norm_coeffs: bad shape");
    if (b == 0) return OGC_OK;
    OGC_REQUIRE(gamma && beta && mean && rstd && a && bb && (stats || (ws && x)), "ogc_group_norm_coeffs: null pointer");
    hipStream_t s = (hipStream_t)stream;
    if (!stats) {
        const int rows = b * groups;
        const long long row_len = (long long)(c / groups) * hw;
        slots = launch_gn_stats(rows, row_len, x, ws, s);
        stats = ws;
    }
    hipLaunchKernelGGL(gn_coeffs_kernel, dim3(ogc_divup(b * c, 256)), dim3(256), 0, s, b, c, hw, groups, eps, gamma, beta,
                       stats, slots, mean, rstd, a, bb);
    OGC_CHECK_LAUNCH("ogc_group_norm_coeffs");
    return OGC_OK;
}

extern "C" int ogc_group_norm_stats_slots(void) { return GN_STATS_SLOTS; }
extern "C" int ogc_group_norm_bwd_slots(void) { return GN_BWD_SLOTS; }

extern "C" int ogc_group_norm_fwd(int b, int c, int hw, int groups, float eps, int relu, const float *x,
                                  const float *gamma, const float *beta, float *y, float *mean, float *rstd,
                                  double *ws, ogc_stream_t stream) {
    return gn_fwd_impl("ogc_group_norm_fwd", b, c, hw, groups, eps, relu, x, gamma, beta, y, mean, rstd, ws, nullptr, 0,
                       stream);
}

extern "C" int ogc_group_norm_fwd_stats(int b, int c, int hw, int groups, float eps, int relu, const float *x,
                                        const float *gamma, const float *beta, float *y, float *mean, float *rstd,
                                        const double *stats, int slots, ogc_stream_t stream) {
    OGC_REQUIRE(stats && slots >= 1, "ogc_group_norm_fwd_stats: no statistics");
    return gn_fwd_impl("ogc_group_norm_fwd_stats", b, c, hw, groups, eps, relu, x, gamma, beta, y, mean, rstd, nullptr,
                       stats, slots, stream);
}

namespace {
template <typename AT>
int gn_bwd_impl(int b, int c, int hw, int groups, int relu, const AT *x, const float *gamma, const float *beta, const float *mean,
                const float *rstd, const AT *grad_y, AT *grad_x, float *grad_gamma, float *grad_beta, double *ws,
                ogc_stream_t stream) {
    OGC_REQUIRE(b >= 0 && c >= 1 && hw >= 1 && groups >= 1 && c % groups == 0, "ogc_group_norm_bwd: bad shape");
    if (b == 0) return OGC_OK;
    if (sizeof(AT) == 2 && ((hw & 3) != 0 || (((uintptr_t)x | (uintptr_t)grad_y | (uintptr_t)grad_x) & 7) != 0)) {
        ogc_set_error("ogc_group_norm_bwd_h: needs hw %% 4 == 0 and 8-byte aligned tensors");
        return OGC_ERR_UNSUPPORTED;
    }
    OGC_REQUIRE(x && gamma && beta && mean && rstd && grad_y && grad_x && grad_gamma && grad_beta && ws,
                "ogc_group_norm_bwd: null pointer");
    hipStream_t s = (hipStream_t)stream;
    double *dsdb = ws;
    dim3 grid(hw_chunks(b, c, hw), c, b);
    const int slots = (int)grid.x;
    if (relu) {
        hipLaunchKernelGGL((gn_bwd_sums_kernel<true, AT>), grid, dim3(GN_THREADS), 0, s, c, hw, groups, x, gamma, beta, mean,
                           rstd, grad_y, dsdb);
        hipLaunchKernelGGL((gn_bwd_dx_kernel<true, AT>), grid, dim3(GN_THREADS), 0, s, c, hw, groups, x, gamma, beta, mean,
                           rstd, dsdb, slots, grad_y, grad_x, grad_gamma, grad_beta);
    } else {
        hipLaunchKernelGGL((gn_bwd_sums_kernel<false, AT>), grid, dim3(GN_THREADS), 0, s, c, hw, groups, x, gamma, beta, mean,
                           rstd, grad_y, dsdb);
        hipLaunchKernelGGL((gn_bwd_dx_kernel<false, AT>), grid, dim3(GN_THREADS), 0, s, c, hw, groups, x, gamma, beta, mean,
                           rstd, dsdb, slots, grad_y, grad_x, grad_gamma, grad_beta);
    }
    OGC_CHECK_LAUNCH("ogc_group_norm_bwd");
    return OGC_OK;
}
}

extern "C" int ogc_group_norm_bwd(int b, int c, int hw, int groups, int relu, const float *x, const float *gamma,
                                  const float *beta, const float *mean, const float *rstd, const float *grad_y,
                                  float *grad_x, float *grad_gamma, float *grad_beta, double *ws,
                                  ogc_stream_t stream) {
    return gn_bwd_impl<float>(b, c, hw, groups, relu, x, gamma, beta, mean, rstd, grad_y, grad_x, grad_gamma, grad_beta, ws, stream);
}

extern "C" int ogc_group_norm_bwd_h(int b, int c, int hw, int groups, int relu, const ogc_bf16_t *x, const float *gamma,
                                    const float *beta, const float *mean, const float *rstd, const ogc_bf16_t *grad_y,
                                    ogc_bf16_t *grad_x, float *grad_gamma, float *grad_beta, double *ws,
                                    ogc_stream_t stream) {
    return gn_bwd_impl<ogc_bf16>(b, c, hw, groups, relu, x, gamma, beta, mean, rstd, grad_y, grad_x, grad_gamma, grad_beta, ws, stream);
}

static bool gn_pool_shape_ok(int s) { return s >= 4 && s <= 256 && (s & (s - 1)) == 0; }

namespace {
int gn_pool_fwd_impl(const char *name, int b, int c, int p, int s, int groups, float eps, int relu, const float *x,
                     const float *gamma, const float *beta, float *out, int *argmax, float *mean, float *rstd,
                     double *ws, const double *stats, int slots, ogc_stream_t stream) {
    OGC_REQUIRE(b >= 0 && c >= 1 && p >= 1 && groups >= 1 && c % groups == 0, "%s: bad shape", name);
    if (!gn_pool_shape_ok(s) || ((uintptr_t)x & 15) != 0) {
        ogc_set_error("%s: nsample=%d must be a power of two in [4,256] and x 16-byte aligned", name, s);
        return OGC_ERR_UNSUPPORTED;
    }
    if (b == 0) return OGC_OK;
    OGC_REQUIRE(x && gamma && beta && out && argmax && mean && rstd && (ws || stats), "%s: null pointer", name);
    OGC_REQUIRE((long long)c * p * s < (1ll << 31) && b <= 65535, "%s: one sample exceeds 32-bit indexing", name);
    hipStream_t st = (hipStream_t)stream;
    if (!stats) {
        const int rows = b * groups;
        const long long row_len = (long long)(c / groups) * p * s;
        slots = launch_gn_stats(rows, row_len, x, ws, st);
        stats = ws;
    }
    const int rows_per_block = GN_THREADS / (s / 4);
    int bx = ogc_divup(p, rows_per_block);
    while (bx > 1 && (long long)bx * c * b > 8192) bx = (bx + 1) / 2;
    dim3 grid(bx, c, b);
    if (relu)
        hipLaunchKernelGGL(gn_apply_maxpool_kernel<true>, grid, dim3(GN_THREADS), 0, st, c, p, s, groups, eps, x, gamma,
                           beta, stats, slots, out, argmax, mean, rstd);
    else
        hipLaunchKernelGGL(gn_apply_maxpool_kernel<false>, grid, dim3(GN_THREADS), 0, st, c, p, s, groups, eps, x,
                           gamma, beta, stats, slots, out, argmax, mean, rstd);
    OGC_CHECK_LAUNCH(name);
    return OGC_OK;
}
}

extern "C" int ogc_group_norm_maxpool_fwd(int b, int c, int p, int s, int groups, float eps, int relu, const float *x,
                                          const float *gamma, const float *beta, float *out, int *argmax,
                                          float *mean, float *rstd, double *ws, ogc_stream_t stream) {
    return gn_pool_fwd_impl("ogc_group_norm_maxpool_fwd", b, c, p, s, groups, eps, relu, x, gamma, beta, out, argmax,
                            mean, rstd, ws, nullptr, 0, stream);
}

extern "C" int ogc_group_norm_maxpool_fwd_stats(int b, int c, int p, int s, int groups, float eps, int relu,
                                                const float *x, const float *gamma, const float *beta, float *out,
                                                int *argmax, float *mean, float *rstd, const double *stats, int slots,
                                                ogc_stream_t stream) {
    OGC_REQUIRE(stats && slots >= 1, "ogc_group_norm_maxpool_fwd_stats: no statistics");
    return gn_pool_fwd_impl("ogc_group_norm_maxpool_fwd_stats", b, c, p, s, groups, eps, relu, x, gamma, beta, out,
                            argmax, mean, rstd, nullptr, stats, slots, stream);
}

extern "C" int ogc_group_norm_pool_extremes(int b, int c, int p, int s, int groups, float eps, int relu,
                                            const float *yext, const int *aext, const float *gamma, const float *beta,
                                            float *out, int *argmax, float *mean, float *rstd, const double *stats,
                                            int slots, ogc_stream_t stream) {
    OGC_REQUIRE(b >= 0 && c >= 1 && p >= 1 && s >= 1 && groups >= 1 && c % groups == 0 && slots >= 1,
                "ogc_group_norm_pool_extremes: bad shape");
    if (b == 0) return OGC_OK;
    OGC_REQUIRE(yext && aext && gamma && beta && out && argmax && mean && rstd && stats,
                "ogc_group_norm_pool_extremes: null pointer");
    OGC_REQUIRE(b <= 65535, "ogc_group_norm_pool_extremes: too many samples for one grid");
    const dim3 grid(c, b);
    hipStream_t st = (hipStream_t)stream;
    if (relu)
        hipLaunchKernelGGL(gn_pool_extremes_kernel<true>, grid, dim3(GN_THREADS), 0, st, c, p, s, groups, eps, yext, aext,
                           gamma, beta, stats, slots, out, argmax, mean, rstd);
    else
        hipLaunchKernelGGL(gn_pool_extremes_kernel<false>, grid, dim3(GN_THREADS), 0, st, c, p, s, groups, eps, yext, aext,
                           gamma, beta, stats, slots, out, argmax, mean, rstd);
    OGC_CHECK_LAUNCH("ogc_group_norm_pool_extremes");
    return OGC_OK;
}

static int gn_maxpool_bwd_impl(int b, int c, int p, int s, int groups, int relu, const float *x, const float *x_at_argmax,
                               const float *gamma, const float *mean, const float *rstd, const float *out,
// ... 110 lines not shown
```

ogc_amd/csrc/ogc_common.h:

```cpp
#pragma once
#include <hip/hip_runtime.h>
#include <stdint.h>

#include "../../include/ogc_ops.h"

#define OGC_WAVE 64

void ogc_set_error(const char *fmt, ...);
void *ogc_workspace(hipStream_t stream, size_t bytes);

#define OGC_REQUIRE(cond, ...)            \
    do {                                  \
        if (!(cond)) {                    \
            ogc_set_error(__VA_ARGS__);   \
            return OGC_ERR_INVALID_ARG;   \
        }                                 \
    } while (0)

#define OGC_CHECK_LAUNCH(name)                                                   \
    do {                                                                         \
        hipError_t e_ = hipGetLastError();                                       \
        if (e_ != hipSuccess) {                                                  \
            ogc_set_error("%s: launch failed: %s", name, hipGetErrorString(e_)); \
            return OGC_ERR_LAUNCH;                                               \
// ... 114 lines not shown
#pragma unroll
    for (int u = 0; u < 4; ++u) dy[u] = q2y - Y[u];
#pragma unroll
    for (int u = 0; u < 4; ++u) dz[u] = q2z - Z[u];
#ifdef OGC_FMAD
#pragma unroll
    for (int u = 0; u < 4; ++u) s[u] = ogc_sqsum3(dx[u], dy[u], dz[u]);
#else
#pragma unroll
    for (int u = 0; u < 4; ++u) dx[u] = dx[u] * dx[u];
#pragma unroll
    for (int u = 0; u < 4; ++u) dy[u] = dy[u] * dy[u];
#pragma unroll
    for (int u = 0; u < 4; ++u) dz[u] = dz[u] * dz[u];
#pragma unroll
    for (int u = 0; u < 4; ++u) s[u] = dx[u] + dy[u];
#pragma unroll
    for (int u = 0; u < 4; ++u) s[u] = s[u] + dz[u];
#endif
#pragma unroll
    for (int u = 0; u < 4; ++u) {
        d[2 * u] = s[u].x;
        d[2 * u + 1] = s[u].y;
    }
}

__device__ __forceinline__ void ogc_tile_fetch(const float *__restrict__ pts, int n, int t, int lane,
                                               float (&r)[8][3]) {
#pragma unroll
    for (int i = 0; i < 8; ++i) {
        const int p = t * OGC_TILE + i * OGC_WAVE + lane;
        if (p < n) {
            const float *q = pts + (size_t)p * 3;
            r[i][0] = q[0]; r[i][1] = q[1]; r[i][2] = q[2];
        } else {
            r[i][0] = r[i][1] = r[i][2] = INFINITY;
        }
    }
}

template <class Group>
__device__ __forceinline__ void ogc_scan_candidates(const float *__restrict__ pts, int n, float qx, float qy,
                                                    float qz, float *tile, int lane, Group &&group) {
    const int ntiles = (n + OGC_TILE - 1) / OGC_TILE;
    float pre[8][3];
    if (ntiles > 0) ogc_tile_fetch(pts, n, 0, lane, pre);
    bool stop = false;
    for (int t = 0; t < ntiles && !stop; ++t) {
#pragma unroll
        for (int i = 0; i < 8; ++i) {
            tile[i * OGC_WAVE + lane] = pre[i][0];
            tile[OGC_TILE + i * OGC_WAVE + lane] = pre[i][1];
            tile[2 * OGC_TILE + i * OGC_WAVE + lane] = pre[i][2];
        }
        if (t + 1 < ntiles) ogc_tile_fetch(pts, n, t + 1, lane, pre);
        const int cnt = min(OGC_TILE, n - t * OGC_TILE);
        const int ngroups = (cnt + 7) >> 3;
        const int base = t * OGC_TILE;
        OgcGroup ga, gb;
        ogc_group_read(tile, 0, ga);
        for (int g = 0; g < ngroups && !stop; g += 2) {
            float d[8];
            ogc_group_read(tile, min(g + 1, OGC_TILE / 8 - 1), gb);
            ogc_dist8(ga, qx, qy, qz, d);
            stop = group(d, base + g * 8);
            if (g + 1 < ngroups && !stop) {
                ogc_group_read(tile, min(g + 2, OGC_TILE / 8 - 1), ga);
                ogc_dist8(gb, qx, qy, qz, d);
                stop = group(d, base + g * 8 + 8);
            }
        }
    }
}

template <int CTRL>
__device__ __forceinline__ float ogc_dpp_f32(float v) {
    return __int_as_float(
        __builtin_amdgcn_update_dpp(0, __float_as_int(v), CTRL, 0xF, 0xF, true));
}
template <int CTRL>
__device__ __forceinline__ unsigned ogc_dpp_u32(unsigned v) {
    return (unsigned)__builtin_amdgcn_update_dpp(0, (int)v, CTRL, 0xF, 0xF, true);
}

__device__ __forceinline__ float ogc_wave_max_f32(float v) {
    v = fmaxf(v, ogc_dpp_f32<0xB1>(v));
    v = fmaxf(v, ogc_dpp_f32<0x4E>(v));
    v = fmaxf(v, ogc_dpp_f32<0x141>(v));
    v = fmaxf(v, ogc_dpp_f32<0x140>(v));
    const int iv = __float_as_int(v);
    const float r0 = __int_as_float(__builtin_amdgcn_readlane(iv, 0));
    const float r1 = __int_as_float(__builtin_amdgcn_readlane(iv, 16));
    const float r2 = __int_as_float(__builtin_amdgcn_readlane(iv, 32));
    const float r3 = __int_as_float(__builtin_amdgcn_readlane(iv, 48));
    return fmaxf(fmaxf(r0, r1), fmaxf(r2, r3));
}
```

ogc_amd/fused.py:

```python
import weakref

import torch
import torch.nn.functional as F
from torch.autograd import Function

from .pointnet2 import pointnet2 as _api



import collections as _collections
import functools as _functools

from .utils.zero_arena import zeroed_empty

GATE_MISSES = _collections.Counter()


def deterministic():
    from . import _lib
    return _lib.DETERMINISTIC

ACT16 = __import__("os").environ.get("OGC_ACT16", "1") != "0"


# ... 605 lines not shown
        nat = _api._native
        mask1, mask2, col12, col21 = ctx.saved_tensors
        PB, N, K = mask1.shape
        gm1, gm2 = torch.empty_like(mask1), torch.empty_like(mask2)
        nat.matched_distance_wrapper(PB, N, K, ctx.p, 1, mask1, mask2, col12, col21, g12.contiguous(), g21.contiguous(),
                                     gm1, gm2)
        return gm1, gm2, None, None, None


@_gate
def matched_distance_available(mask, loss_norm, cross_entropy):
    return (mask.is_cuda and mask.dtype == torch.float32 and not cross_entropy and loss_norm in (1, 2)
            and mask.shape[-1] <= 32 and getattr(_api._native, "matched_distance_wrapper", None) is not None
            and getattr(_api._native, "lsap_maximize_wrapper", None) is not None)


def matched_distances(mask1, mask2, loss_norm):
    nat = _api._native
    mask1, mask2 = mask1.contiguous(), mask2.contiguous()
    PB, N, K = mask1.shape
    dev = mask1.device
    with torch.no_grad():
        counts = zeroed_empty(PB * K * K, torch.int32, dev)
        iou = torch.empty(PB, K, K, dtype=torch.float32, device=dev)
        nat.mask_iou_wrapper(PB, N, K, mask1.detach(), mask2.detach(), counts, iou)
        both = torch.stack([iou, iou.transpose(1, 2)]).contiguous()
        cols = torch.empty(2 * PB, K, dtype=torch.int32, device=dev)
        nat.lsap_maximize_wrapper(2 * PB, K, both, cols)
    return _MatchedDistance.apply(mask1, mask2, cols[:PB], cols[PB:], int(loss_norm))


FUSED_GN_BACKWARD_MAX_WIDTH = 64
FUSED_GN_BACKWARD = True
ACT16_MOMENT_WIDTH = int(__import__("os").environ.get("OGC_ACT16_MOMENT_WIDTH", "64"))


def _moment_width(t):
    return ACT16_MOMENT_WIDTH if t.dtype is torch.bfloat16 else FUSED_GN_BACKWARD_MAX_WIDTH


def _pool_moment_cout(t):
    return ACT16_MOMENT_WIDTH if t.dtype is torch.bfloat16 else max(FUSED_GN_BACKWARD_MAX_WIDTH, SPARSE_POOL_MAX_COUT)


def _norm_act_conv_forward(y_prev, stats_prev, gn_weight, gn_bias, conv_weight, gn_groups, eps, relu, next_groups, pool,
                           next_gamma):
    nat = _api._native
    B, cin = y_prev.shape[0], y_prev.shape[1]
    cout = conv_weight.shape[0]
    hw = y_prev.numel() // (B * cin)
    dev = y_prev.device
    mean = torch.empty(B * gn_groups, dtype=torch.float32, device=dev)
    rstd = torch.empty_like(mean)
    a = torch.empty(B * cin, dtype=torch.float32, device=dev)
    bb = torch.empty_like(a)
    gamma, beta = gn_weight.contiguous(), gn_bias.contiguous()
    if stats_prev is not None:
        nat.group_norm_coeffs_wrapper(B, cin, hw, gn_groups, eps, None, gamma, beta, stats_prev,
                                      stats_prev.numel() // (2 * B * gn_groups), None, mean, rstd, a, bb)
    else:
        ws = nat.group_norm_ws(B, cin, gn_groups, False, dev)
        nat.group_norm_coeffs_wrapper(B, cin, hw, gn_groups, eps, y_prev, gamma, beta, None, 0, ws, mean, rstd, a, bb)
    y = torch.empty((B, cout) + tuple(y_prev.shape[2:]), dtype=y_prev.dtype, device=dev)
    w = conv_weight.contiguous()
    stats = extremes = None
    if (next_groups > 0 and next_groups <= 32 and cout % next_groups == 0 and (cout // next_groups) % 4 == 0
            and (cin <= 100 or _stats_ok(nat, B, cout, cin, hw, True))):
        stats = zeroed_empty(nat.conv1x1_gn_slots() * B * next_groups * 2, torch.float64, dev)
        if (pool and next_gamma is not None and (cin <= 100 or POOL_EXTREMES_WIDE)
                and getattr(nat, "conv1x1_gemm_affine_pool_wrapper", None) is not None):
            centres = hw // pool
            yext = torch.empty(B, cout, centres, dtype=torch.float32, device=dev)
            aext = torch.empty(B, cout, centres, dtype=torch.int32, device=dev)
            nat.conv1x1_gemm_affine_pool_wrapper(B, cout, cin, hw, relu, next_groups, pool, w, y_prev, a, bb,
                                                 next_gamma.contiguous(), y, stats, yext, aext)
            extremes = (yext, aext)
        else:
            nat.conv1x1_gemm_affine_wrapper(B, cout, cin, hw, relu, next_groups, w, y_prev, a, bb, y, stats)
    else:
        nat.conv1x1_gemm_affine_wrapper(B, cout, cin, hw, relu, 0, w, y_prev, a, bb, y, None)
    return y, stats, extremes, mean, rstd, a, bb


class _NormActConv(Function):

    @staticmethod
    def forward(ctx, y_prev, stats_prev, gn_weight, gn_bias, conv_weight, gn_groups, eps, relu, next_groups, pool=0,
                next_gamma=None):
        ctx.set_materialize_grads(False)
        y_prev = y_prev.contiguous()
        y, stats, extremes, mean, rstd, a, bb = _norm_act_conv_forward(y_prev, stats_prev, gn_weight, gn_bias, conv_weight,
                                                                       gn_groups, eps, relu, next_groups, pool, next_gamma)
        hw = y_prev.numel() // (y_prev.shape[0] * y_prev.shape[1])
        ctx.save_for_backward(y_prev, gn_weight, gn_bias, conv_weight, mean, rstd, a, bb)
        ctx.cfg = (gn_groups, relu, hw)
        if extremes is not None:
            ctx.mark_non_differentiable(stats, *extremes)
            return (y, stats) + extremes
        if stats is not None:
            ctx.mark_non_differentiable(stats)
        return y, stats

    @staticmethod
    def backward(ctx, grad_y, _grad_stats=None, *_grad_extremes):
        if grad_y is None:
            return (None,) * 11
        nat = _api._native
        y_prev, gn_weight, gn_bias, conv_weight, mean, rstd, a, bb = ctx.saved_tensors
        gn_groups, relu, hw = ctx.cfg
        B, cin = y_prev.shape[0], y_prev.shape[1]
        cout = conv_weight.shape[0]
        grad_y = grad_y.contiguous()
        w = conv_weight.contiguous()
        grad_w = zeroed_empty((cout, cin), torch.float32, y_prev.device)
        if (FUSED_GN_BACKWARD and getattr(nat, "conv1x1_dgrad_adjoint_wrapper", None) is not None and hw % 64 == 0
                and cout <= _moment_width(y_prev) and cin <= _moment_width(y_prev) and gn_groups <= 32
                and cin % gn_groups == 0):
            dev = y_prev.device
            moments = zeroed_empty((B, 2, cout, cin), torch.float32, dev)
            nat.conv1x1_wgrad_moments_wrapper(B, cin, cout, hw, relu, y_prev, a, bb, grad_y, moments)
            coef = torch.empty(B, cin, 3, dtype=torch.float32, device=dev)
            ggb = zeroed_empty((2, cin), torch.float32, dev)
            gw, gb = ggb[0], ggb[1]
            nat.gn_moments_combine_wrapper(B, cin, cout, hw, gn_groups, moments, w.view(cout, cin), a, bb, mean, rstd,
                                           gn_weight.contiguous(), grad_w, coef, gw, gb)
            grad_prev = torch.empty_like(y_prev)
            nat.conv1x1_dgrad_adjoint_wrapper(B, cin, cout, hw, relu, w.view(cout, cin), grad_y, y_prev, a, bb, coef, grad_prev)
            return grad_prev, None, gw, gb, grad_w.view_as(conv_weight), None, None, None, None, None, None
        nat.conv1x1_wgrad_affine_wrapper(B, cin, cout, hw, relu, y_prev, a, bb, grad_y, grad_w)
        if y_prev.dtype is torch.bfloat16 or (_gemm_ok(cout, hw) and _plain_gemm_mine(cout, (B, cin, hw))):
            grad_z = torch.empty_like(y_prev)
            nat.conv1x1_gemm_wrapper(B, cin, cout, hw, 1, w, grad_y, grad_z)
        else:
            grad_z = _product(w.view(cout, cin), grad_y.reshape(B, cout, hw), True).view_as(y_prev)
        grad_prev = torch.empty_like(y_prev)
        gw, gb = torch.empty_like(gn_weight), torch.empty_like(gn_bias)
        ws = nat.group_norm_ws(B, cin, gn_groups, True, y_prev.device)
        nat.group_norm_bwd_wrapper(B, cin, hw, gn_groups, relu, y_prev, gn_weight.contiguous(),
                                   gn_bias.contiguous(), mean, rstd, grad_z, grad_prev, gw, gb, ws)
        return grad_prev, None, gw, gb, grad_w.view_as(conv_weight), None, None, None, None, None, None


@_gate
def norm_act_conv_available(y_prev, gn, conv):
    if deterministic():
        return False
    if not (y_prev.is_cuda and _is_act(y_prev) and gn.affine and conv.bias is None and conv.groups == 1
            and all(k == 1 for k in conv.kernel_size) and all(v == 1 for v in conv.stride)
            and all(v == 0 for v in conv.padding)
            and getattr(_api._native, "conv1x1_gemm_affine_wrapper", None) is not None):
        return False
    hw = y_prev.numel() // max(y_prev.shape[0] * y_prev.shape[1], 1)
    if y_prev.dtype is torch.bfloat16 and _api._native.get_matmul_precision() != "bf16":
        return False
    return _gemm_ok(y_prev.shape[1], hw)


def act16_middle_ok(y_prev, gn, conv):
    return norm_act_conv_available(y_prev, gn, conv) and conv.weight.shape[0] <= 160


def norm_act_conv(y_prev, stats_prev, gn, relu, conv, next_gn=None, pool=0):
    next_groups = next_gn.num_groups if (next_gn is not None and next_gn.affine) else 0
    res = _NormActConv.apply(y_prev, stats_prev, gn.weight, gn.bias, conv.weight, gn.num_groups, gn.eps, bool(relu),
                             next_groups, int(pool) if (pool in (16, 32, 64) and next_groups) else 0,
                             next_gn.weight if next_groups else None)
    if pool:
        return res[0], res[1], (tuple(res[2:]) if len(res) > 2 else None)
    return res[0], res[1]


SPARSE_POOL_BACKWARD = True
SPARSE_POOL_MAX_COUT = 64
WIDE_POOL_BACKWARD = _os.environ.get("OGC_WIDE_POOL", "1") != "0"

class _NormActConvPool(Function):

    @staticmethod
    def forward(ctx, y_prev, stats_prev, gn_weight, gn_bias, conv_weight, gn_groups, eps, relu, gn2_weight, gn2_bias,
                groups2, eps2, relu2):
        nat = _api._native
        y_prev = y_prev.contiguous()
        B, cin, P, S = y_prev.shape
        cout = conv_weight.shape[0]
        y, stats, extremes, mean, rstd, a, bb = _norm_act_conv_forward(y_prev, stats_prev, gn_weight, gn_bias, conv_weight,
                                                                       gn_groups, eps, relu, groups2, S, gn2_weight)
        dev = y_prev.device
        out = torch.empty(B, cout, P, dtype=torch.float32, device=dev)
        arg = torch.empty(B, cout, P, dtype=torch.int32, device=dev)
        mean2 = torch.empty(B * groups2, dtype=torch.float32, device=dev)
        rstd2 = torch.empty_like(mean2)
        g2, b2 = gn2_weight.contiguous(), gn2_bias.contiguous()
        nat.group_norm_pool_extremes_wrapper(B, cout, P, S, groups2, eps2, relu2, extremes[0], extremes[1], g2, b2, out, arg,
                                             mean2, rstd2, stats, stats.numel() // (2 * B * groups2))
        ctx.save_for_backward(y_prev, gn_weight, gn_bias, conv_weight, mean, rstd, a, bb, y, gn2_weight, mean2, rstd2, out, arg,
                              extremes[0])
        ctx.cfg = (gn_groups, relu, groups2, relu2)
        return out

    @staticmethod
    def backward(ctx, grad_out):
        nat = _api._native
        (y_prev, gn_weight, gn_bias, conv_weight, mean, rstd, a, bb, y, gn2_weight, mean2, rstd2, out, arg,
         yext) = ctx.saved_tensors
        gn_groups, relu, groups2, relu2 = ctx.cfg
        B, cin, P, S = y_prev.shape
        cout, hw, dev = conv_weight.shape[0], P * S, y_prev.device
        coef2 = torch.empty(B, cout, 2, dtype=torch.float32, device=dev)
        inj = torch.empty(B, cout, P, 2, dtype=torch.float32, device=dev)
        gw2, gb2 = torch.empty_like(gn2_weight), torch.empty_like(gn2_weight)
        ws = nat.group_norm_ws(B, cout, groups2, True, dev)
        nat.group_norm_maxpool_bwd_sparse_wrapper(B, cout, P, S, groups2, relu2, y, gn2_weight.contiguous(), mean2,
                                                  rstd2, out, arg, grad_out.contiguous(), coef2, inj, gw2, gb2, ws,
                                                  yext if POOL_SUMS_FROM_EXTREMES else None)
        w = conv_weight.contiguous().view(cout, cin)
        if cin > _moment_width(y_prev) or cout > _pool_moment_cout(y_prev):
            grad_w = zeroed_empty((cout, cin), torch.float32, dev)
            nat.conv1x1_wgrad_affine_pooled_wrapper(B, cin, cout, hw, relu, S, y_prev, a, bb, y, coef2, inj, grad_w)
            grad_z = torch.empty_like(y_prev)
            nat.conv1x1_dgrad_pooled_wrapper(B, cin, cout, hw, S, w, y, coef2, inj, grad_z)
            grad_prev = torch.empty_like(y_prev)
            gw, gb = torch.empty_like(gn_weight), torch.empty_like(gn_bias)
            ws = nat.group_norm_ws(B, cin, gn_groups, True, dev)
            nat.group_norm_bwd_wrapper(B, cin, hw, gn_groups, relu, y_prev, gn_weight.contiguous(), gn_bias.contiguous(), mean,
                                       rstd, grad_z, grad_prev, gw, gb, ws)
            return (grad_prev, None, gw, gb, grad_w.view_as(conv_weight), None, None, None, gw2, gb2, None, None, None)
        moments = zeroed_empty((B, 2, cout, cin), torch.float32, dev)
        nat.conv1x1_wgrad_moments_pooled_wrapper(B, cin, cout, hw, relu, S, y_prev, a, bb, y, coef2, inj, moments)
        coef = torch.empty(B, cin, 3, dtype=torch.float32, device=dev)
        ggb = zeroed_empty((2, cin), torch.float32, dev)
        gw, gb = ggb[0], ggb[1]
        grad_w = torch.empty(cout, cin, dtype=torch.float32, device=dev)
        nat.gn_moments_combine_wrapper(B, cin, cout, hw, gn_groups, moments, w, a, bb, mean, rstd,
                                       gn_weight.contiguous(), grad_w, coef, gw, gb)
        grad_prev = torch.empty_like(y_prev)
        nat.conv1x1_dgrad_adjoint_pooled_wrapper(B, cin, cout, hw, relu, S, w, y, coef2, inj, y_prev, a, bb, coef, grad_prev)
        return (grad_prev, None, gw, gb, grad_w.view_as(conv_weight), None, None, None, gw2, gb2, None, None, None)


@_gate
def norm_act_conv_pool_available(y_prev, gn, conv, next_gn):
    nat = _api._native
    if not (SPARSE_POOL_BACKWARD and FUSED_GN_BACKWARD and y_prev.dim() == 4 and y_prev.shape[-1] in (16, 32, 64)
            and next_gn is not None and next_gn.affine and norm_act_conv_available(y_prev, gn, conv)
            and getattr(nat, "conv1x1_dgrad_adjoint_pooled_wrapper", None) is not None
            and getattr(nat, "conv1x1_gemm_affine_pool_wrapper", None) is not None):
        return False
    cin, cout, g, g2 = y_prev.shape[1], conv.weight.shape[0], gn.num_groups, next_gn.num_groups
    if cin > _moment_width(y_prev) or cout > _pool_moment_cout(y_prev):
        B, hw = y_prev.shape[0], y_prev.shape[2] * y_prev.shape[3]
        return (WIDE_POOL_BACKWARD and getattr(nat, "conv1x1_dgrad_pooled_wrapper", None) is not None
                and hw % 64 == 0 and B * (hw // 64) >= 1024 and B <= 65535
                and g <= 32 and cin % g == 0 and g2 <= 32 and cout % g2 == 0 and (cout // g2) % 4 == 0
                and (cin <= 100 or (POOL_EXTREMES_WIDE and _stats_ok(nat, B, cout, cin, hw, True))))
    kq = (cout + 3) // 4
    lds = (64 * 4 * (kq | 1) + 320) * 4 + 4 * cout * (64 // y_prev.shape[-1]) * 16
    return (lds <= 65536 and (y_prev.shape[2] * y_prev.shape[3]) % 64 == 0 and cin <= _moment_width(y_prev)
            and cout <= _pool_moment_cout(y_prev) and g <= 32 and cin % g == 0
            and g2 <= 32 and cout % g2 == 0 and (cout // g2) % 4 == 0)


def norm_act_conv_pool(y_prev, stats_prev, gn, relu, conv, next_gn, next_relu):
    return _NormActConvPool.apply(y_prev, stats_prev, gn.weight, gn.bias, conv.weight, gn.num_groups, gn.eps, bool(relu),
                                  next_gn.weight, next_gn.bias, next_gn.num_groups, next_gn.eps, bool(next_relu))


class _SelfAttentionCore(Function):

    @staticmethod
    def forward(ctx, qkv, n_head):
        nat = _api._native
        qkv = qkv.contiguous()
        B, L, E3 = qkv.shape
        E = E3 // 3
        out = torch.empty(B, L, E, dtype=torch.float32, device=qkv.device)
        prob = torch.empty(B, n_head, L, L, dtype=torch.float32, device=qkv.device)
        scale = (E // n_head) ** -0.5
        nat.attention_fwd_wrapper(n_head, scale, qkv[:, :, :E], qkv[:, :, E:2 * E], qkv[:, :, 2 * E:], out, prob)
        ctx.save_for_backward(qkv, out, prob)
        ctx.cfg = (n_head, scale)
        return out

    @staticmethod
    def backward(ctx, grad_out):
        qkv, out, prob = ctx.saved_tensors
        n_head, scale = ctx.cfg
        E = qkv.shape[2] // 3
        grad = torch.empty_like(qkv)
        _api._native.attention_bwd_wrapper(n_head, scale, qkv[:, :, :E], qkv[:, :, E:2 * E], qkv[:, :, 2 * E:], out, prob,
                                           grad_out.contiguous(), grad[:, :, :E], grad[:, :, E:2 * E], grad[:, :, 2 * E:])
        return grad, None


class _CrossAttentionCore(Function):

    @staticmethod
    def forward(ctx, q, kv, n_head):
        nat = _api._native
        q, kv = q.contiguous(), kv.contiguous()
        B, Lq, E = q.shape
        Lk = kv.shape[1]
        out = torch.empty(B, Lq, E, dtype=torch.float32, device=q.device)
# ... 274 lines not shown
```

ogc_amd/pointnet2_cuda.py:

```python
import torch

from . import _lib


def _check(t, dtype, name):
    try:
        if t.is_cuda and t.dtype is dtype and t.is_contiguous():
            return t.data_ptr()
    except AttributeError:
        pass
    if not isinstance(t, torch.Tensor):
        raise TypeError("%s must be a torch.Tensor" % name)
    if t.device.type != "cuda":
        raise RuntimeError("%s must be a CUDA tensor (HIP device); ogc_amd has no CPU path" % name)
    if not t.is_contiguous():
        raise RuntimeError("%s must be contiguous" % name)
    if t.dtype != dtype:
        raise RuntimeError("%s must be %s, got %s" % (name, dtype, t.dtype))
    return t.data_ptr()


def _f(t, name):
    return _check(t, torch.float32, name)

# ... 298 lines not shown


def group_linear_fwd_pt_wrapper(b, m, n, npoints, nsample, groups, Pt, idx, rel, wx, y, stats):
    _run("ogc_group_linear_fwd_pt_h", Pt, b, m, n, npoints, nsample, int(groups), _f(Pt, "Pt"), _i(idx, "idx"), _f(rel, "rel"),
         _f(wx, "wx"), _check(y, torch.bfloat16, "y"), _opt(stats, torch.float64, "stats"))


def group_linear_fwd_direct_wrapper(b, m, cf, n, npoints, nsample, groups, feats, idx, rel, w, y, stats):
    h, (yp,) = _acts((y,), ("y",))
    _run("ogc_group_linear_fwd_direct" + h, feats, b, m, cf, n, npoints, nsample, int(groups), _f(feats, "feats"), _i(idx, "idx"),
         _f(rel, "rel"), _f(w, "w"), yp, _opt(stats, torch.float64, "stats"))


def group_linear_bwd_wrapper(b, m, n, npoints, nsample, grad_y, idx, rel, grad_p, dwx):
    _run("ogc_group_linear_bwd", grad_y, b, m, n, npoints, nsample, _f(grad_y, "grad_y"), _i(idx, "idx"), _f(rel, "rel"),
         _f(grad_p, "grad_p"), _f(dwx, "dwx"))


def soft_nn_target_wrapper(b, n1, n2, k, temperature, p1, p2, mask1, mask2, target):
    _run("ogc_soft_nn_target", p1, b, n1, n2, k, float(temperature), _f(p1, "p1"), _f(p2, "p2"), _f(mask1, "mask1"),
         _f(mask2, "mask2"), _f(target, "target"))


def rigid_moments_wrapper(vb, n, k, pc, pc2, mask, mom, S, means):
    _run("ogc_rigid_moments", pc, vb, n, k, _f(pc, "pc"), _f(pc2, "pc2"), _f(mask, "mask"),
         _check(mom, torch.float64, "mom"), _f(S, "S"), _f(means, "means"))


def rigid_translation_wrapper(total, means, valid, R, t):
    _run("ogc_rigid_translation", means, total, _f(means, "means"), _i(valid, "valid"), _f(R, "R"), _f(t, "t"))


def rigid_blend_wrapper(vb, n, k, p, backward, pc, pc2, mask, R, t, grad_out, out):
    _run("ogc_rigid_blend", pc, vb, n, k, int(p), int(backward), _f(pc, "pc"), _f(pc2, "pc2"), _f(mask, "mask"),
         _f(R, "R"), _f(t, "t"), 0 if grad_out is None else _f(grad_out, "grad_out"), _f(out, "out"))


def mask_iou_wrapper(pb, n, k, mask1, mask2, counts, iou):
    _run("ogc_mask_iou", mask1, pb, n, k, _f(mask1, "mask1"), _f(mask2, "mask2"), _i(counts, "counts"), _f(iou, "iou"))


def matched_distance_wrapper(pb, n, k, p, backward, mask1, mask2, col12, col21, grad12, grad21, out1, out2):
    _run("ogc_matched_distance", mask1, pb, n, k, int(p), int(backward), _f(mask1, "mask1"), _f(mask2, "mask2"),
         _i(col12, "col12"), _i(col21, "col21"), 0 if grad12 is None else _f(grad12, "grad12"),
         0 if grad21 is None else _f(grad21, "grad21"), _f(out1, "out1"), _f(out2, "out2"))


def lsap_maximize_wrapper(np_, k, score, col4row):
    _run("ogc_lsap_maximize", score, np_, k, _f(score, "score"), _i(col4row, "col4row"))


def sym_eigvals_wrapper(nb, k, A, w):
    _run("ogc_sym_eigvals", A, nb, k, _check(A, torch.float64, "A"), _check(w, torch.float64, "w"))


def neighbour_consistency_fwd_wrapper(b, n, c, k, p, mask, idx, out):
    _run("ogc_neighbour_consistency_fwd", mask, b, n, c, k, int(p), _f(mask, "mask"), _i(idx, "idx"), _f(out, "out"))


def reverse_neighbours_wrapper(b, n, k, idx, rev_start, rev_src, rev_mult, ws):
    _run("ogc_reverse_neighbours", idx, b, n, k, _i(idx, "idx"), _i(rev_start, "rev_start"), _i(rev_src, "rev_src"),
         _i(rev_mult, "rev_mult"), _i(ws, "ws"))


def neighbour_consistency_bwd_wrapper(b, n, c, k, p, mask, idx, rev_start, rev_src, rev_mult, grad_out, grad_mask):
    _run("ogc_neighbour_consistency_bwd", mask, b, n, c, k, int(p), _f(mask, "mask"), _i(idx, "idx"),
         _i(rev_start, "rev_start"), _i(rev_src, "rev_src"), _i(rev_mult, "rev_mult"), _f(grad_out, "grad_out"),
         _f(grad_mask, "grad_mask"))


def group_norm_fwd_wrapper(b, c, hw, groups, eps, relu, x, gamma, beta, y, mean, rstd, ws):
    _run("ogc_group_norm_fwd", x, b, c, hw, groups, float(eps), int(relu), _f(x, "x"), _f(gamma, "gamma"),
         _f(beta, "beta"), _f(y, "y"), _f(mean, "mean"), _f(rstd, "rstd"), _check(ws, torch.float64, "ws"))


def group_norm_bwd_wrapper(b, c, hw, groups, relu, x, gamma, beta, mean, rstd, grad_y, grad_x, grad_gamma, grad_beta,
                           ws):
    h, (xp, gyp, gxp) = _acts((x, grad_y, grad_x), ("x", "grad_y", "grad_x"))
    _run("ogc_group_norm_bwd" + h, x, b, c, hw, groups, int(relu), xp, _f(gamma, "gamma"), _f(beta, "beta"),
         _f(mean, "mean"), _f(rstd, "rstd"), gyp, gxp,
         _f(grad_gamma, "grad_gamma"), _f(grad_beta, "grad_beta"), _check(ws, torch.float64, "ws"))


def group_norm_maxpool_fwd_wrapper(b, c, p, s, groups, eps, relu, x, gamma, beta, out, argmax, mean, rstd, ws):
    _run("ogc_group_norm_maxpool_fwd", x, b, c, p, s, groups, float(eps), int(relu), _f(x, "x"), _f(gamma, "gamma"),
         _f(beta, "beta"), _f(out, "out"), _i(argmax, "argmax"), _f(mean, "mean"), _f(rstd, "rstd"),
         _check(ws, torch.float64, "ws"))


def group_norm_maxpool_bwd_wrapper(b, c, p, s, groups, relu, x, gamma, mean, rstd, out, argmax, grad_out, grad_x,
                                   grad_gamma, grad_beta, ws):
    _run("ogc_group_norm_maxpool_bwd", x, b, c, p, s, groups, int(relu), _f(x, "x"), _f(gamma, "gamma"),
         _f(mean, "mean"), _f(rstd, "rstd"), _f(out, "out"), _i(argmax, "argmax"), _f(grad_out, "grad_out"),
         _f(grad_x, "grad_x"), _f(grad_gamma, "grad_gamma"), _f(grad_beta, "grad_beta"),
         _check(ws, torch.float64, "ws"))


def group_norm_maxpool_bwd_ext_wrapper(b, c, p, s, groups, relu, x, x_at_argmax, gamma, mean, rstd, out, argmax, grad_out,
                                       grad_x, grad_gamma, grad_beta, ws):
    _run("ogc_group_norm_maxpool_bwd_ext", x, b, c, p, s, groups, int(relu), _f(x, "x"), _f(x_at_argmax, "x_at_argmax"),
         _f(gamma, "gamma"), _f(mean, "mean"), _f(rstd, "rstd"), _f(out, "out"), _i(argmax, "argmax"),
         _f(grad_out, "grad_out"), _f(grad_x, "grad_x"), _f(grad_gamma, "grad_gamma"), _f(grad_beta, "grad_beta"),
         _check(ws, torch.float64, "ws"))


def conv1x1_wgrad_wrapper(b, cin, cout, hw, x, dy, dw):
    if dy.dtype is torch.bfloat16:
        _run("ogc_conv1x1_wgrad_xf_h", x, b, cin, cout, hw, _f(x, "x"), _check(dy, torch.bfloat16, "dy"), _f(dw, "dw"))
        return
    _run("ogc_conv1x1_wgrad", x, b, cin, cout, hw, _f(x, "x"), _f(dy, "dy"), _f(dw, "dw"))


def _opt(t, dtype, name):
    return 0 if t is None else _check(t, dtype, name)


def batch_norm_fwd_wrapper(b, c, hw, eps, relu, training, momentum, x, gamma, beta, running_mean, running_var, y, mean,
                           rstd, ws, stats, slots):
    _run("ogc_batch_norm_fwd", x, b, c, hw, float(eps), int(relu), int(training), float(momentum), _f(x, "x"),
         _f(gamma, "gamma"), _f(beta, "beta"), _opt(running_mean, torch.float32, "running_mean"),
         _opt(running_var, torch.float32, "running_var"), _f(y, "y"), _opt(mean, torch.float32, "mean"),
         _opt(rstd, torch.float32, "rstd"), _opt(ws, torch.float64, "ws"), _opt(stats, torch.float64, "stats"), int(slots))


def batch_norm_bwd_wrapper(b, c, hw, relu, training, x, gamma, beta, mean, rstd, grad_y, grad_x, grad_gamma, grad_beta,
                           ws):
    _run("ogc_batch_norm_bwd", x, b, c, hw, int(relu), int(training), _f(x, "x"), _f(gamma, "gamma"), _f(beta, "beta"),
         _f(mean, "mean"), _f(rstd, "rstd"), _f(grad_y, "grad_y"), _f(grad_x, "grad_x"), _f(grad_gamma, "grad_gamma"),
         _f(grad_beta, "grad_beta"), _check(ws, torch.float64, "ws"))


def batch_norm_maxpool_fwd_wrapper(b, c, p, s, eps, relu, training, momentum, x, gamma, beta, running_mean, running_var,
                                   out, argmax, mean, rstd, ws, stats, slots):
    _run("ogc_batch_norm_maxpool_fwd", x, b, c, p, s, float(eps), int(relu), int(training), float(momentum), _f(x, "x"),
         _f(gamma, "gamma"), _f(beta, "beta"), _opt(running_mean, torch.float32, "running_mean"),
         _opt(running_var, torch.float32, "running_var"), _f(out, "out"), _i(argmax, "argmax"),
         _opt(mean, torch.float32, "mean"), _opt(rstd, torch.float32, "rstd"), _opt(ws, torch.float64, "ws"),
         _opt(stats, torch.float64, "stats"), int(slots))


def batch_norm_maxpool_bwd_wrapper(b, c, p, s, relu, training, x, gamma, mean, rstd, out, argmax, grad_out, grad_x,
                                   grad_gamma, grad_beta, ws):
    _run("ogc_batch_norm_maxpool_bwd", x, b, c, p, s, int(relu), int(training), _f(x, "x"), _f(gamma, "gamma"),
         _f(mean, "mean"), _f(rstd, "rstd"), _f(out, "out"), _i(argmax, "argmax"), _f(grad_out, "grad_out"),
         _f(grad_x, "grad_x"), _f(grad_gamma, "grad_gamma"), _f(grad_beta, "grad_beta"), _check(ws, torch.float64, "ws"))


def group_norm_coeffs_wrapper(b, c, hw, groups, eps, x, gamma, beta, stats, slots, ws, mean, rstd, a, bb):
    _run("ogc_group_norm_coeffs", gamma, b, c, hw, groups, float(eps), _opt(x, torch.float32, "x"), _f(gamma, "gamma"),
         _f(beta, "beta"), _opt(stats, torch.float64, "stats"), int(slots), _opt(ws, torch.float64, "ws"),
         _f(mean, "mean"), _f(rstd, "rstd"), _f(a, "a"), _f(bb, "bb"))


def conv1x1_gemm_affine_wrapper(b, M, K, hw, relu, groups, w, inp, pa, pb, out, stats):
    h, (ip, op) = _acts((inp, out), ("in", "out"))
    _run("ogc_conv1x1_gemm_affine" + h, inp, b, M, K, hw, int(relu), int(groups), _f(w, "w"), ip, _f(pa, "pa"),
         _f(pb, "pb"), op, _opt(stats, torch.float64, "stats"))


def conv1x1_gemm_affine_pool_wrapper(b, M, K, hw, relu, groups, nsample, w, inp, pa, pb, next_gamma, out, stats, yext,
                                     aext):
    h, (ip, op) = _acts((inp, out), ("in", "out"))
    _run("ogc_conv1x1_gemm_affine_pool" + h, inp, b, M, K, hw, int(relu), int(groups), int(nsample), _f(w, "w"),
         ip, _f(pa, "pa"), _f(pb, "pb"), _f(next_gamma, "next_gamma"), op,
         _check(stats, torch.float64, "stats"), _f(yext, "yext"), _i(aext, "aext"))

# ... 116 lines not shown
def slot_masks_fwd_wrapper(temperature, feats, slots, mask):
    b, d, n = feats.shape
    _run("ogc_slot_masks_fwd", feats, b, d, n, slots.shape[2], float(temperature), _f(feats, "feats"),
         _f(slots, "slots"), _f(mask, "mask"))


def slot_masks_bwd_wrapper(temperature, feats, slots, mask, grad_mask, grad_feats, grad_slots):
    b, d, n = feats.shape
    k = slots.shape[2]
    ws = torch.empty(max(int(_lib.load().ogc_slot_masks_ws_floats(b, d, n, k)), 1), dtype=torch.float32,
                     device=feats.device)
    _run("ogc_slot_masks_bwd", feats, b, d, n, k, float(temperature), _f(feats, "feats"), _f(slots, "slots"),
         _f(mask, "mask"), _f(grad_mask, "grad_mask"), _f(grad_feats, "grad_feats"), _f(grad_slots, "grad_slots"),
         _f(ws, "ws"))


def group_norm_ws(b, c, groups, backward, device):
    L = _lib.load()
    n = 2 * b * c * L.ogc_group_norm_bwd_slots() if backward else 2 * b * groups * L.ogc_group_norm_stats_slots()
    return torch.empty(max(n, 1), dtype=torch.float64, device=device)


_precision = "fp32"


def set_matmul_precision(mode):
    global _precision
    if mode not in ("fp32", "bf16"):
        raise ValueError("matmul precision must be 'fp32' or 'bf16'")
    previous = "bf16" if _lib.load().ogc_set_matmul_precision(1 if mode == "bf16" else 0) else "fp32"
    _precision = mode
    return previous


def get_matmul_precision():
    return _precision


def conv1x1_gemm_stream_supported(b, m, k, hw):
    return bool(_lib.load().ogc_conv1x1_gemm_stream_supported(int(b), int(m), int(k), int(hw)))


def conv1x1_gemm_stats_supported(b, m, k, hw, affine):
    return bool(_lib.load().ogc_conv1x1_gemm_stats_supported(int(b), int(m), int(k), int(hw), 1 if affine else 0))


def conv1x1_gn_slots():
    return _lib.load().ogc_conv1x1_gn_slots()


def conv1x1_gemm_gnstats_wrapper(b, M, K, hw, groups, w, inp, out, stats):
    _run("ogc_conv1x1_gemm_gnstats", inp, b, M, K, hw, groups, _f(w, "w"), _f(inp, "in"), _f(out, "out"),
         _check(stats, torch.float64, "stats"))


def group_norm_fwd_stats_wrapper(b, c, hw, groups, eps, relu, x, gamma, beta, y, mean, rstd, stats, slots):
    _run("ogc_group_norm_fwd_stats", x, b, c, hw, groups, float(eps), int(relu), _f(x, "x"), _f(gamma, "gamma"),
         _f(beta, "beta"), _f(y, "y"), _f(mean, "mean"), _f(rstd, "rstd"), _check(stats, torch.float64, "stats"),
         int(slots))


def group_norm_maxpool_fwd_stats_wrapper(b, c, p, s, groups, eps, relu, x, gamma, beta, out, argmax, mean, rstd, stats,
                                         slots):
    _run("ogc_group_norm_maxpool_fwd_stats", x, b, c, p, s, groups, float(eps), int(relu), _f(x, "x"),
         _f(gamma, "gamma"), _f(beta, "beta"), _f(out, "out"), _i(argmax, "argmax"), _f(mean, "mean"),
         _f(rstd, "rstd"), _check(stats, torch.float64, "stats"), int(slots))


def conv1x1_gemm_wrapper(b, M, K, hw, transpose_a, w, inp, out):
    h, (ip, op) = _acts((inp, out), ("in", "out"))
    _run("ogc_conv1x1_gemm" + h, inp, b, M, K, hw, int(transpose_a), _f(w, "w"), ip, op)


def conv1x1_gemm_any_wrapper(b, M, K, hw, transpose_a, w, inp, out):
    _run("ogc_conv1x1_gemm_any", inp, b, M, K, hw, int(transpose_a), _f(w, "w"), _f(inp, "in"), _f(out, "out"))


def conv1x1_wgrad_affine_pooled_wrapper(b, cin, cout, hw, relu, nsample, x, pa, pb, y, coef2, inj, dw):
    h, (xp, yp) = _acts((x, y), ("x", "y"))
    _run("ogc_conv1x1_wgrad_affine_pooled" + h, x, b, cin, cout, hw, int(relu), nsample, xp, _f(pa, "pa"), _f(pb, "pb"),
         yp, _f(coef2, "coef2"), _f(inj, "inj"), _f(dw, "dw"))


def conv1x1_dgrad_pooled_wrapper(b, cin, cout, hw, nsample, w, y, coef2, inj, grad_z):
    h, (yp, gp) = _acts((y, grad_z), ("y", "grad_z"))
    _run("ogc_conv1x1_dgrad_pooled" + h, y, b, cin, cout, hw, nsample, _f(w, "w"), yp, _f(coef2, "coef2"), _f(inj, "inj"), gp)
```

Before: 1568 point-clouds/s.

## Fuse GroupNorm backward reduction sums into conv1x1 input-gradient GEMM epilogue

The conv1x1 dgrad kernels (plain streaming and pooled) now compute, in their epilogue, the per-channel GroupNorm backward sums (dy*x and dy, with ReLU masking) while the gradient tile is still in registers. They accumulate these in double precision in LDS and flush them to slotted global partials. A new group_norm_bwd_dx kernel then consumes those partials to form grad_x, grad_gamma and grad_beta, so the GroupNorm backward no longer needs its own reduction pass over grad_z and x. The cost is extra loads of the pre-norm activation, double-precision DPP reductions and atomics inside the GEMM epilogue, and more LDS, which may reduce occupancy.

```diff
diff --git a/include/ogc_ops.h b/include/ogc_ops.h
--- a/include/ogc_ops.h
+++ b/include/ogc_ops.h
@@ -15,7 +15,7 @@
     OGC_ERR_UNSUPPORTED = -3
 };
 
-#define OGC_VERSION 205
+#define OGC_VERSION 206
 int ogc_version(void);
 int ogc_distance_contracted(void);
 int ogc_set_deterministic(int on);
@@ -255,6 +255,18 @@
                                     ogc_stream_t stream);
 int ogc_conv1x1_dgrad_pooled(int b, int cin, int cout, int hw, int nsample, const float *w, const float *y, const float *coef2,
                              const float *inj, float *grad_z, ogc_stream_t stream);
+
+int ogc_group_norm_bwd_dx(int b, int c, int hw, int groups, int relu, const float *x, const float *gamma, const float *beta,
+                          const float *mean, const float *rstd, const float *grad_y, const double *dsdb, int slots,
+                          float *grad_x, float *grad_gamma, float *grad_beta, ogc_stream_t stream);
+int ogc_conv1x1_dgrad_pooled_gnsums(int b, int cin, int cout, int hw, int nsample, int groups, int relu, const float *w,
+                                    const float *y, const float *coef2, const float *inj, const float *y_prev,
+                                    const float *gamma, const float *beta, const float *mean, const float *rstd,
+                                    float *grad_z, double *dsdb, ogc_stream_t stream);
+int ogc_conv1x1_dgrad_gnsums_supported(int b, int cin, int cout, int hw);
+int ogc_conv1x1_dgrad_gnsums(int b, int cin, int cout, int hw, int relu, const float *w, const float *grad_y,
+                             const float *y_prev, const float *gamma, const float *beta, const float *mean, const float *rstd,
+                             int groups, float *grad_z, double *dsdb, ogc_stream_t stream);
 
 int ogc_group_norm_fwd_stats(int b, int c, int hw, int groups, float eps, int relu, const float *x,
                              const float *gamma, const float *beta, float *y, float *mean, float *rstd,
diff --git a/ogc_amd/_lib.py b/ogc_amd/_lib.py
--- a/ogc_amd/_lib.py
+++ b/ogc_amd/_lib.py
@@ -113,6 +113,11 @@
     "ogc_conv1x1_wgrad_affine": [_int, _int, _int, _int, _int, _vp, _vp, _vp, _vp, _vp, _vp],
     "ogc_conv1x1_wgrad_affine_pooled": [_int, _int, _int, _int, _int, _int, _vp, _vp, _vp, _vp, _vp, _vp, _vp, _vp],
     "ogc_conv1x1_dgrad_pooled": [_int, _int, _int, _int, _int, _vp, _vp, _vp, _vp, _vp, _vp],
+    "ogc_group_norm_bwd_dx": [_int, _int, _int, _int, _int, _vp, _vp, _vp, _vp, _vp, _vp, _vp, _int, _vp, _vp, _vp, _vp],
+    "ogc_conv1x1_dgrad_pooled_gnsums": [_int, _int, _int, _int, _int, _int, _int, _vp, _vp, _vp, _vp, _vp, _vp, _vp, _vp, _vp,
+                                        _vp, _vp, _vp],
+    "ogc_conv1x1_dgrad_gnsums_supported": [_int, _int, _int, _int],
+    "ogc_conv1x1_dgrad_gnsums": [_int, _int, _int, _int, _int, _vp, _vp, _vp, _vp, _vp, _vp, _vp, _int, _vp, _vp, _vp],
     "ogc_batch_norm_fwd": [_int, _int, _int, _flt, _int, _int, _flt, _vp, _vp, _vp, _vp, _vp, _vp, _vp, _vp, _vp, _vp,
                            _int, _vp],
     "ogc_batch_norm_bwd": [_int, _int, _int, _int, _int, _vp, _vp, _vp, _vp, _vp, _vp, _vp, _vp, _vp, _vp, _vp],
@@ -139,7 +144,7 @@
 SIGNATURES["ogc_conv1x1_wgrad_xf_h"] = SIGNATURES["ogc_conv1x1_wgrad"]
 SIGNATURES["ogc_group_linear_fwd_pt_h"] = SIGNATURES["ogc_group_linear_fwd"]
 
-HEADER_VERSION = 205
+HEADER_VERSION = 206
 _lib = None
 _fns = {}
 
diff --git a/ogc_amd/csrc/conv1x1.hip b/ogc_amd/csrc/conv1x1.hip
--- a/ogc_amd/csrc/conv1x1.hip
+++ b/ogc_amd/csrc/conv1x1.hip
@@ -238,7 +238,8 @@
     }
 }
 
-template <int KQ, bool PRO, bool EXACT, bool STATS = false, bool POOL = false, bool DUAL = false, bool TRANS = false>
+template <int KQ, bool PRO, bool EXACT, bool STATS = false, bool POOL = false, bool DUAL = false, bool TRANS = false,
+          bool GNS = false>
 __global__ __launch_bounds__(WG_WAVES *OGC_WAVE, DUAL ? 2 : 1) void conv1x1_gemm_stream_kernel(int M, int K, int hw, int ntiles,
                                                                                  const float *__restrict__ w,
                                                                                  const float *__restrict__ in,
@@ -247,7 +248,9 @@
                                                                                  const float *__restrict__ pb, int pro_relu,
                                                                                  int groups = 1, int nbatch = 1,
                                                                                  double *__restrict__ stats = nullptr,
-                                                                                 PoolOut pool = PoolOut()) {
+                                                                                 PoolOut pool = PoolOut(),
+                                                                                 OgcGnSums gn = OgcGnSums()) {
+    static_assert(!GNS || (!STATS && !PRO && !POOL), "GroupNorm sums: the plain input gradient only");
     extern __shared__ __attribute__((aligned(16))) float a_lds[];
     const int lane = threadIdx.x & 63, wave = __builtin_amdgcn_readfirstlane(threadIdx.x >> 6);
     const int j = lane & 15, kk = lane >> 4;
@@ -259,8 +262,25 @@
     if constexpr (POOL) {
         for (int t = threadIdx.x; t < Mt * 64; t += WG_WAVES * OGC_WAVE) sgn_all[t] = (t < M && pool.sign[t] < 0.f) ? -1.f : 1.f;
     }
+    const int nw = gridDim.x * WG_WAVES;
+    double *gacc = reinterpret_cast<double *>(a_lds + (size_t)Mt * 64 * a_ld);
+    float2 *gcoef = reinterpret_cast<float2 *>(gacc + 4 * M);
+    int gn_b0 = 0, gn_b1 = -1;
+    if constexpr (GNS) {
+        const int per_wg = WG_WAVES * ((ntiles + nw - 1) / nw);
+        const int first = blockIdx.x * per_wg, last = min(ntiles, first + per_wg) - 1;
+        if (first <= last) { gn_b0 = first / tiles_per_img; gn_b1 = last / tiles_per_img; }
+        for (int e = threadIdx.x; e < 2 * M; e += WG_WAVES * OGC_WAVE) {
+            const int bs = min(gn_b0 + e / M, nbatch - 1), ch = e % M;
+            const int cg = M / gn.groups, row = bs * gn.groups + ch / cg;
+            const float a = gn.rstd[row] * gn.gamma[ch];
+            const float bb = gn.beta[ch] - gn.mean[row] * a;
+            gcoef[e] = make_float2(a, bb);
+            gacc[2 * e] = 0.0;
+            gacc[2 * e + 1] = 0.0;
+        }
+    }
     __syncthreads();
-    const int nw = gridDim.x * WG_WAVES;
     const unsigned off_main = (unsigned)(kk * hw + 4 * j);
     const unsigned off_last = (unsigned)(min(kk, K - 1 - (Kq - 1) * 4) * hw + 4 * j);
     auto load_tile = [&](int t, float4(&x)[KQ]) {
@@ -324,9 +344,21 @@
         }
         float *outb = out + (size_t)b * M * hw + p0;
         const unsigned off_out = (unsigned)(kk * 4 * hw + 4 * j);
+        const float *gxb = GNS ? gn.x + (size_t)b * M * hw + p0 : nullptr;
+        const int gset = GNS ? (b - gn_b0) * M : 0;
+        auto load_gx = [&](int mt, int a, float4(&v)[4]) {
+#pragma unroll
+            for (int r = 0; r < 4; ++r) {
+                const int m0 = mt * 64 + a * 16 + r;
+                v[r] = EXACT ? *reinterpret_cast<const float4 *>(gxb + (size_t)m0 * hw + off_out)
+                             : *reinterpret_cast<const float4 *>(gxb + (size_t)min(m0 + kk * 4, M - 1) * hw + 4 * j);
+            }
+        };
         for (int mt = 0; mt < Mt; ++mt) {
             const float *at = a_lds + (size_t)mt * 64 * a_ld;
             const int nblk = EXACT ? 4 : min(4, (M - mt * 64 + 15) >> 4);
+            float4 gx[2][4];
+            if constexpr (GNS) load_gx(mt, 0, gx[0]);
             v4f acc[4][4];
 #pragma unroll
             for (int a = 0; a < 4; ++a)
@@ -350,14 +382,40 @@
                 }
             }
 #pragma unroll
-            for (int a = 0; a < 4; ++a)
+            for (int a = 0; a < 4; ++a) {
+                if constexpr (GNS) {
+                    if (a < 3) load_gx(mt, a + 1, gx[(a + 1) & 1]);
+                }
 #pragma unroll
                 for (int r = 0; r < 4; ++r) {
                     const int m0 = mt * 64 + a * 16 + r;
                     if (EXACT || m0 + kk * 4 < M)
                         *reinterpret_cast<float4 *>(outb + (size_t)m0 * hw + off_out) =
                             make_float4(acc[a][0][r], acc[a][1][r], acc[a][2][r], acc[a][3][r]);
-                }
+                    if constexpr (GNS) {
+                        const int m = m0 + kk * 4;
+                        const bool ok = EXACT || m < M;
+                        const float2 cf = gcoef[gset + (EXACT ? m : min(m, M - 1))];
+                        const float4 v = gx[a & 1][r];
+                        float4 d = make_float4(acc[a][0][r], acc[a][1][r], acc[a][2][r], acc[a][3][r]);
+                        if (gn.relu) {
+                            const float ca = cf.x, cb = cf.y;
+                            d.x = fmaf(ca, v.x, cb) > 0.f ? d.x : 0.f; d.y = fmaf(ca, v.y, cb) > 0.f ? d.y : 0.f;
+                            d.z = fmaf(ca, v.z, cb) > 0.f ? d.z : 0.f; d.w = fmaf(ca, v.w, cb) > 0.f ? d.w : 0.f;
+                        }
+                        double s = ok ? (double)((d.x * v.x + d.y * v.y) + (d.z * v.z + d.w * v.w)) : 0.0;
+                        double sb = ok ? (double)((d.x + d.y) + (d.z + d.w)) : 0.0;
+                        s += ogc_dpp_f64<0xB1>(s); sb += ogc_dpp_f64<0xB1>(sb);
+                        s += ogc_dpp_f64<0x4E>(s); sb += ogc_dpp_f64<0x4E>(sb);
+                        s += ogc_dpp_f64<0x141>(s); sb += ogc_dpp_f64<0x141>(sb);
+                        s += ogc_dpp_f64<0x140>(s); sb += ogc_dpp_f64<0x140>(sb);
+                        if (j == 0 && ok) {
+                            __hip_atomic_fetch_add(gacc + 2 * (gset + m), s, __ATOMIC_RELAXED, __HIP_MEMORY_SCOPE_WORKGROUP);
+                            __hip_atomic_fetch_add(gacc + 2 * (gset + m) + 1, sb, __ATOMIC_RELAXED, __HIP_MEMORY_SCOPE_WORKGROUP);
+                        }
+                    }
+                }
+            }
             if constexpr (POOL) {
                 const int m0p = mt * 64;
                 const int centres = hw / pool.s;
@@ -395,6 +453,16 @@
             }
         }
     };
+    auto flush_gn = [&]() {
+        if constexpr (GNS) {
+            __syncthreads();
+            double *dst = gn.dsdb + (size_t)(blockIdx.x % gn.slots) * nbatch * M * 2;
+            for (int e = threadIdx.x; e < 4 * M; e += WG_WAVES * OGC_WAVE) {
+                const int bs = gn_b0 + e / (2 * M);
+                if (bs <= gn_b1) unsafeAtomicAdd(dst + (size_t)bs * M * 2 + e % (2 * M), gacc[e]);
+            }
+        }
+    };
     const int per = (ntiles + nw - 1) / nw;
     int t = (blockIdx.x * WG_WAVES + wave) * per;
     const int t_end = min(ntiles, t + per);
@@ -406,6 +474,7 @@
             compute_store(t, x1);
         }
         if (STATS) flush_stats();
+        flush_gn();
         return;
     }
     float4 xa[KQ], xb[KQ];
@@ -420,6 +489,7 @@
         if (t < t_end) compute_store(t, xa);
     }
     if (STATS) flush_stats();
+    flush_gn();
 }
 
 bool gemm_stream_eligible(int b, int M, int K, int hw, bool pro, bool pool = false, bool any_precision = false) {
@@ -432,30 +502,37 @@
              ntiles >= (1ll << 31));
 }
 
-template <bool PRO, bool STATS = false, bool POOL = false, bool TRANS = false>
+template <bool PRO, bool STATS = false, bool POOL = false, bool TRANS = false, bool GNS = false>
 bool gemm_stream_launch(int b, int M, int K, int hw, const float *w, const float *in, float *out, const float *pa,
                         const float *pb, int pro_relu, hipStream_t s, int groups = 1, double *stats = nullptr,
-                        PoolOut pool = PoolOut()) {
+                        PoolOut pool = PoolOut(), OgcGnSums gn = OgcGnSums(), bool dry = false) {
     const int Kq = (K + 3) / 4, Mt = (M + 63) / 64;
     const long long ntiles = (long long)b * (hw / 64);
+    const size_t strip = WG_WAVES * 4 * 16 * 2 * sizeof(double), gns_strip = (size_t)M * (2 * 2 * sizeof(double) + 2 * sizeof(float2));
     const size_t lds = ((size_t)Mt * 64 * ogc_a_ld(Kq) + (PRO ? WG_WAVES * 2 * FW_KQ_MAX * 4 : 0)) * sizeof(float) +
-                       WG_WAVES * 4 * 16 * 2 * sizeof(double) + (POOL ? (size_t)Mt * 64 * sizeof(float) : 0);
+                       ((GNS && gns_strip > strip) ? gns_strip : strip) + (POOL ? (size_t)Mt * 64 * sizeof(float) : 0);
     if (!gemm_stream_eligible(b, M, K, hw, PRO, POOL, STATS) || lds > 156 * 1024) return false;
     const int wgs = (int)(ntiles / WG_WAVES < 256 ? ntiles / WG_WAVES : 256);
 #define OGC_STREAM_D(KQV, EX, DU, WGS)                                                                                       \
     do {                                                                                                                     \
         static bool raised = false;                                                                                          \
-        const void *fn = reinterpret_cast<const void *>(&conv1x1_gemm_stream_kernel<KQV, PRO, EX, STATS, POOL, DU, TRANS>);         \
+        const void *fn = reinterpret_cast<const void *>(&conv1x1_gemm_stream_kernel<KQV, PRO, EX, STATS, POOL, DU, TRANS, GNS>);    \
         if (!raised) {                                                                                                       \
             if (hipFuncSetAttribute(fn, hipFuncAttributeMaxDynamicSharedMemorySize, 156 * 1024) != hipSuccess) return false;  \
             raised = true;                                                                                                   \
         }                                                                                                                    \
-        hipLaunchKernelGGL((conv1x1_gemm_stream_kernel<KQV, PRO, EX, STATS, POOL, DU, TRANS>), dim3(WGS), dim3(WG_WAVES * OGC_WAVE), \
-                           lds, s, M, K, hw, (int)ntiles, w, in, out, pa, pb, pro_relu, groups, b, stats, pool);             \
+        hipLaunchKernelGGL((conv1x1_gemm_stream_kernel<KQV, PRO, EX, STATS, POOL, DU, TRANS, GNS>), dim3(WGS),               \
+                           dim3(WG_WAVES * OGC_WAVE), lds, s, M, K, hw, (int)ntiles, w, in, out, pa, pb, pro_relu, groups, b, stats, \
+                           pool, gn);                                                                                        \
     } while (0)
     static const bool dual_on = !(getenv("OGC_GEMM_STREAM_DUAL") && getenv("OGC_GEMM_STREAM_DUAL")[0] == '0');
     const bool dual = dual_on && !POOL && 2 * (lds + 1024) <= 156 * 1024 && ntiles >= 4096;
     const int wgs2 = (int)(ntiles / WG_WAVES < 512 ? ntiles / WG_WAVES : 512);
+    if (GNS) {
+        const long long nw = (long long)(dual ? wgs2 : wgs) * WG_WAVES;
+        if (WG_WAVES * ((ntiles + nw - 1) / nw) > hw / 64) return false;
+    }
+    if (dry) return true;
 #define OGC_STREAM(KQV, EX)                                                                                                  \
     do {                                                                                                                     \
         if (dual) OGC_STREAM_D(KQV, EX, true, wgs2);                                                                         \
@@ -576,6 +653,42 @@
     return (K <= 100 || g_matmul_bf16 || gemm_stream_eligible(b, M, K, hw, affine != 0, false, true)) ? 1 : 0;
 }
 
+extern "C" int ogc_conv1x1_dgrad_gnsums_supported(int b, int cin, int cout, int hw) {
+    if (b < 1 || cin < 1 || cout < 1 || hw < 1) return 0;
+    return gemm_stream_launch<false, false, false, true, true>(b, cin, cout, hw, nullptr, nullptr, nullptr, nullptr, nullptr, 0,
+                                                               nullptr, 1, nullptr, PoolOut(), OgcGnSums(), true) ? 1 : 0;
+}
+
+extern "C" int ogc_conv1x1_dgrad_gnsums(int b, int cin, int cout, int hw, int relu, const float *w, const float *grad_y,
+                                        const float *y_prev, const float *gamma, const float *beta, const float *mean,
+                                        const float *rstd, int groups, float *grad_z, double *dsdb, ogc_stream_t stream) {
+    const char *name = "ogc_conv1x1_dgrad_gnsums";
+    const int rc = gemm_check(name, b, cin, cout, hw, w, grad_y, grad_z);
+    if (rc != OGC_OK) return rc;
+    OGC_REQUIRE(y_prev && gamma && beta && mean && rstd && dsdb, "%s: null pointer", name);
+    OGC_REQUIRE(groups >= 1 && cin % groups == 0, "%s: bad group count", name);
+    if (((uintptr_t)y_prev & 15) != 0 || !ogc_conv1x1_dgrad_gnsums_supported(b, cin, cout, hw)) {
+        if (b == 0) return OGC_OK;
+        ogc_set_error("%s: not a shape of the streaming kernel (ogc_conv1x1_dgrad_gnsums_supported), or y_prev misaligned", name);
+        return OGC_ERR_UNSUPPORTED;
+    }
+    hipStream_t s = (hipStream_t)stream;
+    OgcGnSums gn;
+    gn.x = y_prev; gn.gamma = gamma; gn.beta = beta; gn.mean = mean; gn.rstd = rstd; gn.dsdb = dsdb;
+    gn.groups = groups; gn.relu = relu; gn.slots = ogc_group_norm_bwd_slots();
+    if (ogc_zero_async(dsdb, (size_t)gn.slots * b * cin * 2 * sizeof(double), s) != hipSuccess) {
+        ogc_set_error("%s: clearing the partial sums failed", name);
+        return OGC_ERR_LAUNCH;
+    }
+    if (!gemm_stream_launch<false, false, false, true, true>(b, cin, cout, hw, w, grad_y, grad_z, nullptr, nullptr, 0, s, 1, nullptr,
+                                                             PoolOut(), gn)) {
+        ogc_set_error("%s: the streaming kernel refused the launch", name);
+        return OGC_ERR_LAUNCH;
+    }
+    OGC_CHECK_LAUNCH(name);
+    return OGC_OK;
+}
+
 extern "C" int ogc_conv1x1_gemm_stream_supported(int b, int M, int K, int hw) {
     if (b < 1 || M < 1 || K < 1 || hw < 1) return 0;
     return gemm_stream_eligible(b, M, K, hw, false) ? 1 : 0;
diff --git a/ogc_amd/csrc/conv1x1_shared.h b/ogc_amd/csrc/conv1x1_shared.h
--- a/ogc_amd/csrc/conv1x1_shared.h
+++ b/ogc_amd/csrc/conv1x1_shared.h
@@ -20,3 +20,9 @@
     u.h[1] = __builtin_convertvector((v2f){c, d}, v2bf);
     return u.s;
 }
+
+struct OgcGnSums {
+    const float *x = nullptr, *gamma = nullptr, *beta = nullptr, *mean = nullptr, *rstd = nullptr;
+    double *dsdb = nullptr;
+    int groups = 1, relu = 0, slots = 1;
+};
diff --git a/ogc_amd/csrc/gemm_chunk.hip b/ogc_amd/csrc/gemm_chunk.hip
--- a/ogc_amd/csrc/gemm_chunk.hip
+++ b/ogc_amd/csrc/gemm_chunk.hip
@@ -11,17 +11,20 @@
 __device__ __forceinline__ v4s gc_pack_bf16(float a, float b, float c, float d) { return ogc_pack_bf16_rr(a, b, c, d); }
 
 template <int RB, int KQ, bool SPLIT_M, bool TRANS, bool POOLED = false, int KA = 1, typename AT = float, bool BF = false,
-          bool TAB = false>
+          bool TAB = false, bool GNS = false>
 __global__ __launch_bounds__(GC_WAVES *OGC_WAVE, 2) void gemm_chunk_kernel(int M, int K, int hw, const float *__restrict__ w,
                                                                          const AT *__restrict__ in,
                                                                          AT *__restrict__ out,
                                                                          const float2 *__restrict__ coef2 = nullptr,
                                                                          const float2 *__restrict__ inj = nullptr,
-                                                                         int s_shift = 0) {
+                                                                         int s_shift = 0, OgcGnSums gs = OgcGnSums()) {
     constexpr int KC = 4 * KQ, KCA = KC * KA, LD = 4 * ((KQ * KA) | 1);
     constexpr int MT = SPLIT_M ? 64 * RB : 16 * RB;
     constexpr int PER = (MT * KCA) / (GC_WAVES * OGC_WAVE);
     static_assert((MT * KCA) % (GC_WAVES * OGC_WAVE) == 0 && PER >= 1 && (KA == 1 || KA == 2), "staging split");
+    static_assert(!GNS || (POOLED && !SPLIT_M && sizeof(AT) == 4 && MT <= GC_WAVES * OGC_WAVE &&
+                           GC_WAVES * MT * 2 * sizeof(double) <= 2 * MT * LD * sizeof(float)),
+                  "GroupNorm sums: fp32 pooled input gradient; the partial sums of the four wavefronts fit the weights' buffers");
     extern __shared__ __attribute__((aligned(16))) float gc_lds[];
     const int t = threadIdx.x, lane = t & 63, wave = __builtin_amdgcn_readfirstlane(t >> 6);
     const int j = lane & 15, kk = lane >> 4;
@@ -76,6 +79,16 @@
             tab[e] = make_float4(c2v.x, c2v.y, jj.x, jj.y);
         }
         __builtin_amdgcn_wave_barrier();
+    }
+    float2 *gcoef = reinterpret_cast<float2 *>(gc_lds + 2 * MT * LD + ((POOLED && TAB) ? GC_WAVES * K * cpw * 4 : 0));
+    if constexpr (GNS) {
+        if (t < MT) {
+            const int ch = min(m0 + t, M - 1);
+            const int cg = M / gs.groups, row = b * gs.groups + ch / cg;
+            const float a = gs.rstd[row] * gs.gamma[ch];
+            const float bb = gs.beta[ch] - gs.mean[row] * a;
+            gcoef[t] = make_float2(a, bb);
+        }
     }
     const int mine_c = (4 * j) >> s_shift;
     auto load_in = [&](int k0, float4(&xv)[KQ], float2(&cc)[NP], float2(&jv)[NP]) {
@@ -198,15 +211,55 @@
         if (more2) store_a(buf0, a_next);
         __syncthreads();
     }
-    if (!active) return;
-    AT *ob = out + (size_t)b * M * hw + p0 + 4 * j;
+    if (!GNS && !active) return;
+    AT *ob = out + (size_t)b * M * hw + pl + 4 * j;
 #pragma unroll
     for (int a = 0; a < RB; ++a) {
-        if (a < nblk) {
+        if (active && a < nblk) {
 #pragma unroll
             for (int r = 0; r < 4; ++r) {
                 const int m = m0 + wrow + a * 16 + kk * 4 + r;
                 if (m < M) ogc_st4(ob + (size_t)m * hw, make_float4(acc[a][0][r], acc[a][1][r], acc[a][2][r], acc[a][3][r]));
+            }
+        }
+    }
+    if constexpr (GNS) {
+        double *red = reinterpret_cast<double *>(gc_lds);
+        const float *xb = gs.x + (size_t)b * M * hw + pl + 4 * j;
+#pragma unroll
+        for (int a = 0; a < RB; ++a) {
+            float4 xv[4];
+#pragma unroll
+            for (int r = 0; r < 4; ++r) xv[r] = ogc_ld4(xb + (size_t)min(m0 + a * 16 + kk * 4 + r, M - 1) * hw);
+#pragma unroll
+            for (int r = 0; r < 4; ++r) {
+                const int lr = a * 16 + kk * 4 + r;
+                const float2 cf = gcoef[lr];
+                const float4 v = xv[r];
+                float4 d = make_float4(acc[a][0][r], acc[a][1][r], acc[a][2][r], acc[a][3][r]);
+                if (gs.relu) {
+                    const float ca = cf.x, cb = cf.y;
+                    d.x = fmaf(ca, v.x, cb) > 0.f ? d.x : 0.f; d.y = fmaf(ca, v.y, cb) > 0.f ? d.y : 0.f;
+                    d.z = fmaf(ca, v.z, cb) > 0.f ? d.z : 0.f; d.w = fmaf(ca, v.w, cb) > 0.f ? d.w : 0.f;
+                }
+                const bool ok = active && m0 + lr < M;
+                double s = ok ? (double)((d.x * v.x + d.y * v.y) + (d.z * v.z + d.w * v.w)) : 0.0;
+                double sb = ok ? (double)((d.x + d.y) + (d.z + d.w)) : 0.0;
+                s += ogc_dpp_f64<0xB1>(s); sb += ogc_dpp_f64<0xB1>(sb);
+                s += ogc_dpp_f64<0x4E>(s); sb += ogc_dpp_f64<0x4E>(sb);
+                s += ogc_dpp_f64<0x141>(s); sb += ogc_dpp_f64<0x141>(sb);
+                s += ogc_dpp_f64<0x140>(s); sb += ogc_dpp_f64<0x140>(sb);
+                if (j == 0) *reinterpret_cast<double2 *>(red + ((size_t)wave * MT + lr) * 2) = make_double2(s, sb);
+            }
+        }
+        __syncthreads();
+        double *dst = gs.dsdb + (((size_t)(blockIdx.x % gs.slots) * gridDim.z + b) * M + m0) * 2;
+        for (int e = t; e < 2 * MT; e += GC_WAVES * OGC_WAVE) {
+            if (m0 + (e >> 1) < M) {
+                double v = red[e];
+#pragma unroll
+                for (int wv = 1; wv < GC_WAVES; ++wv) v += red[(size_t)wv * MT * 2 + e];
+                unsafeAtomicAdd(dst + e, v);
             }
         }
     }
@@ -274,60 +327,87 @@
 
 namespace {
 template <typename AT>
-int dgrad_pooled_impl(int b, int cin, int cout, int hw, int nsample, const float *w, const AT *y, const float *coef2,
-                      const float *inj, AT *grad_z, ogc_stream_t stream) {
+int dgrad_pooled_impl(const char *name, int b, int cin, int cout, int hw, int nsample, const float *w, const AT *y, const float *coef2,
+                      const float *inj, AT *grad_z, ogc_stream_t stream, const OgcGnSums *gs = nullptr) {
     constexpr bool BF = sizeof(AT) == 2;
-    OGC_REQUIRE(b >= 0 && cin >= 1 && cout >= 1 && hw >= 1, "ogc_conv1x1_dgrad_pooled: bad shape");
-    OGC_REQUIRE(w && y && coef2 && inj && grad_z, "ogc_conv1x1_dgrad_pooled: null pointer");
+    constexpr bool F32 = sizeof(AT) == 4;
+    OGC_REQUIRE(b >= 0 && cin >= 1 && cout >= 1 && hw >= 1, "%s: bad shape", name);
+    OGC_REQUIRE(w && y && coef2 && inj && grad_z, "%s: null pointer", name);
+    if (gs) {
+        OGC_REQUIRE(gs->groups >= 1 && cin % gs->groups == 0, "%s: bad group count", name);
+        OGC_REQUIRE(gs->x && gs->gamma && gs->beta && gs->mean && gs->rstd && gs->dsdb, "%s: null pointer", name);
+    }
     const int sh = nsample == 16 ? 4 : nsample == 32 ? 5 : nsample == 64 ? 6 : -1;
     if (sh < 0 || hw % nsample != 0 || (hw & 63) != 0 || (long long)b * (hw / 64) < 1024 ||
-        (((uintptr_t)y | (uintptr_t)grad_z) & ogc_act_mask<AT>()) != 0 || (((uintptr_t)coef2 | (uintptr_t)inj) & 7) != 0 ||
-        (BF && !ogc_g_matmul_bf16)) {
-        ogc_set_error("ogc_conv1x1_dgrad_pooled: needs nsample in {16, 32, 64} dividing hw, hw %% 64 == 0, >= 1024 tiles of 64 "
-                      "positions and aligned tensors (hw=%d, nsample=%d, b=%d)", hw, nsample, b);
+        (((uintptr_t)y | (uintptr_t)grad_z | (uintptr_t)(gs ? gs->x : nullptr)) & ogc_act_mask<AT>()) != 0 ||
+        (((uintptr_t)coef2 | (uintptr_t)inj) & 7) != 0 || (BF && !ogc_g_matmul_bf16)) {
+        ogc_set_error("%s: needs nsample in {16, 32, 64} dividing hw, hw %% 64 == 0, >= 1024 tiles of 64 "
+                      "positions and aligned tensors (hw=%d, nsample=%d, b=%d)", name, hw, nsample, b);
         return OGC_ERR_UNSUPPORTED;
     }
     OGC_REQUIRE((long long)cin * hw < (1ll << 31) && (long long)cout * hw < (1ll << 31) && b <= 65535,
-                "ogc_conv1x1_dgrad_pooled: one sample exceeds 32-bit indexing");
+                "%s: one sample exceeds 32-bit indexing", name);
     if (b == 0) return OGC_OK;
     hipStream_t s = (hipStream_t)stream;
     const float2 *c2 = reinterpret_cast<const float2 *>(coef2), *ij = reinterpret_cast<const float2 *>(inj);
     const int M = cin, K = cout;
+    if (gs && ogc_zero_async(gs->dsdb, (size_t)gs->slots * b * M * 2 * sizeof(double), s) != hipSuccess) {
+        ogc_set_error("%s: clearing the partial sums failed", name);
+        return OGC_ERR_LAUNCH;
+    }
     static const bool tab_off = [] { const char *e = getenv("OGC_DGRAD_POOLED_TAB"); return e && e[0] == '0'; }();
     const size_t tab_bytes = (size_t)GC_WAVES * K * (64 >> sh) * sizeof(float4);
     const bool tab = !tab_off && tab_bytes <= 24 * 1024;
+#define GC_POOLED(RBV, KQV, KAV, TABV, GNSV)                                                                                       \
+    hipLaunchKernelGGL((gemm_chunk_kernel<RBV, KQV, false, true, true, KAV, AT, BF, TABV, GNSV>), grid, dim3(GC_WAVES * OGC_WAVE), \
+                       lds + (TABV ? tab_bytes : 0) + (GNSV ? 16 * RBV * sizeof(float2) : 0), s, M, K, hw, w, y, grad_z, c2, ij,   \
+                       sh, GNSV ? *gs : OgcGnSums())
     if (M <= 64) {
         constexpr int RB = 4, KQ = 4, KA = 2;
         dim3 grid(ogc_divup(hw, 64 * GC_WAVES), ogc_divup(M, 16 * RB), b);
         const size_t lds = (size_t)2 * 16 * RB * 4 * ((KQ * KA) | 1) * sizeof(float);
-        if (tab)
-            hipLaunchKernelGGL((gemm_chunk_kernel<RB, KQ, false, true, true, KA, AT, BF, true>), grid, dim3(GC_WAVES * OGC_WAVE),
-                               lds + tab_bytes, s, M, K, hw, w, y, grad_z, c2, ij, sh);
-        else
-            hipLaunchKernelGGL((gemm_chunk_kernel<RB, KQ, false, true, true, KA, AT, BF>), grid, dim3(GC_WAVES * OGC_WAVE), lds, s, M,
-                               K, hw, w, y, grad_z, c2, ij, sh);
+        if (gs) {
+            if constexpr (F32) {
+                if (tab) GC_POOLED(RB, KQ, KA, true, true);
+                else GC_POOLED(RB, KQ, KA, false, true);
+            }
+        } else if (tab) GC_POOLED(RB, KQ, KA, true, false);
+        else GC_POOLED(RB, KQ, KA, false, false);
     } else {
         constexpr int RB = 8, KQ = 4;
         dim3 grid(ogc_divup(hw, 64 * GC_WAVES), ogc_divup(M, 16 * RB), b);
         const size_t lds = (size_t)2 * 16 * RB * 4 * (KQ | 1) * sizeof(float);
-        if (tab)
-            hipLaunchKernelGGL((gemm_chunk_kernel<RB, KQ, false, true, true, 1, AT, BF, true>), grid, dim3(GC_WAVES * OGC_WAVE),
-                               lds + tab_bytes, s, M, K, hw, w, y, grad_z, c2, ij, sh);
-        else
-            hipLaunchKernelGGL((gemm_chunk_kernel<RB, KQ, false, true, true, 1, AT, BF>), grid, dim3(GC_WAVES * OGC_WAVE), lds, s, M, K,
-                               hw, w, y, grad_z, c2, ij, sh);
-    }
-    OGC_CHECK_LAUNCH("ogc_conv1x1_dgrad_pooled");
+        if (gs) {
+            if constexpr (F32) {
+                if (tab) GC_POOLED(RB, KQ, 1, true, true);
+                else GC_POOLED(RB, KQ, 1, false, true);
+            }
+        } else if (tab) GC_POOLED(RB, KQ, 1, true, false);
+        else GC_POOLED(RB, KQ, 1, false, false);
+    }
+#undef GC_POOLED
+    OGC_CHECK_LAUNCH(name);
     return OGC_OK;
 }
 }
 
 extern "C" int ogc_conv1x1_dgrad_pooled(int b, int cin, int cout, int hw, int nsample, const float *w, const float *y,
                                         const float *coef2, const float *inj, float *grad_z, ogc_stream_t stream) {
-    return dgrad_pooled_impl<float>(b, cin, cout, hw, nsample, w, y, coef2, inj, grad_z, stream);
+    return dgrad_pooled_impl<float>("ogc_conv1x1_dgrad_pooled", b, cin, cout, hw, nsample, w, y, coef2, inj, grad_z, stream);
+}
+
+extern "C" int ogc_conv1x1_dgrad_pooled_gnsums(int b, int cin, int cout, int hw, int nsample, int groups, int relu, const float *w,
+                                               const float *y, const float *coef2, const float *inj, const float *y_prev,
+                                               const float *gamma, const float *beta, const float *mean, const float *rstd,
+                                               float *grad_z, double *dsdb, ogc_stream_t stream) {
+    OgcGnSums gs;
+    gs.x = y_prev; gs.gamma = gamma; gs.beta = beta; gs.mean = mean; gs.rstd = rstd; gs.dsdb = dsdb;
+    gs.groups = groups; gs.relu = relu; gs.slots = ogc_group_norm_bwd_slots();
+    return dgrad_pooled_impl<float>("ogc_conv1x1_dgrad_pooled_gnsums", b, cin, cout, hw, nsample, w, y, coef2, inj, grad_z, stream,
+                                    &gs);
 }
 
 extern "C" int ogc_conv1x1_dgrad_pooled_h(int b, int cin, int cout, int hw, int nsample, const float *w, const ogc_bf16_t *y,
                                           const float *coef2, const float *inj, ogc_bf16_t *grad_z, ogc_stream_t stream) {
-    return dgrad_pooled_impl<ogc_bf16>(b, cin, cout, hw, nsample, w, y, coef2, inj, grad_z, stream);
-}
+    return dgrad_pooled_impl<ogc_bf16>("ogc_conv1x1_dgrad_pooled_h", b, cin, cout, hw, nsample, w, y, coef2, inj, grad_z, stream);
+}
diff --git a/ogc_amd/csrc/group_norm.hip b/ogc_amd/csrc/group_norm.hip
--- a/ogc_amd/csrc/group_norm.hip
+++ b/ogc_amd/csrc/group_norm.hip
@@ -596,6 +596,28 @@
     return gn_bwd_impl<float>(b, c, hw, groups, relu, x, gamma, beta, mean, rstd, grad_y, grad_x, grad_gamma, grad_beta, ws, stream);
 }
 
+extern "C" int ogc_group_norm_bwd_dx(int b, int c, int hw, int groups, int relu, const float *x, const float *gamma,
+                                     const float *beta, const float *mean, const float *rstd, const float *grad_y,
+                                     const double *dsdb, int slots, float *grad_x, float *grad_gamma, float *grad_beta,
+                                     ogc_stream_t stream) {
+    OGC_REQUIRE(b >= 0 && c >= 1 && hw >= 1 && groups >= 1 && c % groups == 0 && slots >= 1 && slots <= GN_BWD_SLOTS,
+                "ogc_group_norm_bwd_dx: bad shape");
+    if (b == 0) return OGC_OK;
+    OGC_REQUIRE(x && gamma && beta && mean && rstd && grad_y && dsdb && grad_x && grad_gamma && grad_beta,
+                "ogc_group_norm_bwd_dx: null pointer");
+    OGC_REQUIRE(b <= 65535 && c <= 65535, "ogc_group_norm_bwd_dx: too many samples or channels for one grid");
+    hipStream_t s = (hipStream_t)stream;
+    dim3 grid(hw_chunks(b, c, hw), c, b);
+    if (relu)
+        hipLaunchKernelGGL((gn_bwd_dx_kernel<true, float>), grid, dim3(GN_THREADS), 0, s, c, hw, groups, x, gamma, beta, mean, rstd,
+                           dsdb, slots, grad_y, grad_x, grad_gamma, grad_beta);
+    else
+        hipLaunchKernelGGL((gn_bwd_dx_kernel<false, float>), grid, dim3(GN_THREADS), 0, s, c, hw, groups, x, gamma, beta, mean, rstd,
+                           dsdb, slots, grad_y, grad_x, grad_gamma, grad_beta);
+    OGC_CHECK_LAUNCH("ogc_group_norm_bwd_dx");
+    return OGC_OK;
+}
+
 extern "C" int ogc_group_norm_bwd_h(int b, int c, int hw, int groups, int relu, const ogc_bf16_t *x, const float *gamma,
                                     const float *beta, const float *mean, const float *rstd, const ogc_bf16_t *grad_y,
                                     ogc_bf16_t *grad_x, float *grad_gamma, float *grad_beta, double *ws,
diff --git a/ogc_amd/csrc/ogc_common.h b/ogc_amd/csrc/ogc_common.h
--- a/ogc_amd/csrc/ogc_common.h
+++ b/ogc_amd/csrc/ogc_common.h
@@ -220,6 +220,12 @@
 __device__ __forceinline__ unsigned ogc_dpp_u32(unsigned v) {
     return (unsigned)__builtin_amdgcn_update_dpp(0, (int)v, CTRL, 0xF, 0xF, true);
 }
+template <int CTRL>
+__device__ __forceinline__ double ogc_dpp_f64(double v) {
+    const int lo = __builtin_amdgcn_update_dpp(0, __double2loint(v), CTRL, 0xF, 0xF, true);
+    const int hi = __builtin_amdgcn_update_dpp(0, __double2hiint(v), CTRL, 0xF, 0xF, true);
+    return __hiloint2double(hi, lo);
+}
 
 __device__ __forceinline__ float ogc_wave_max_f32(float v) {
     v = fmaxf(v, ogc_dpp_f32<0xB1>(v));
diff --git a/ogc_amd/fused.py b/ogc_amd/fused.py
--- a/ogc_amd/fused.py
+++ b/ogc_amd/fused.py
@@ -711,6 +711,17 @@
     return y, stats, extremes, mean, rstd, a, bb
 
 
+GN_SUMS_IN_DGRAD = True
+
+
+def _gn_bwd_dx(nat, B, cin, hw, gn_groups, relu, y_prev, gn_weight, gn_bias, mean, rstd, grad_z, dsdb):
+    grad_prev = torch.empty_like(y_prev)
+    gw, gb = torch.empty_like(gn_weight), torch.empty_like(gn_bias)
+    nat.group_norm_bwd_dx_wrapper(B, cin, hw, gn_groups, relu, y_prev, gn_weight.contiguous(), gn_bias.contiguous(), mean, rstd,
+                                  grad_z, dsdb, nat.group_norm_bwd_slots(), grad_prev, gw, gb)
+    return grad_prev, gw, gb
+
+
 class _NormActConv(Function):
 
     @staticmethod
@@ -757,6 +768,16 @@
             nat.conv1x1_dgrad_adjoint_wrapper(B, cin, cout, hw, relu, w.view(cout, cin), grad_y, y_prev, a, bb, coef, grad_prev)
             return grad_prev, None, gw, gb, grad_w.view_as(conv_weight), None, None, None, None, None, None
         nat.conv1x1_wgrad_affine_wrapper(B, cin, cout, hw, relu, y_prev, a, bb, grad_y, grad_w)
+        if (GN_SUMS_IN_DGRAD and y_prev.dtype is torch.float32 and grad_y.dtype is torch.float32 and DGRAD_STREAM
+                and cin % gn_groups == 0 and nat.get_matmul_precision() == "fp32"
+                and getattr(nat, "conv1x1_dgrad_gnsums_wrapper", None) is not None
+                and nat.conv1x1_dgrad_gnsums_supported(B, cin, cout, hw)):
+            grad_z = torch.empty_like(y_prev)
+            dsdb = zeroed_empty(2 * B * cin * nat.group_norm_bwd_slots(), torch.float64, y_prev.device)
+            nat.conv1x1_dgrad_gnsums_wrapper(B, cin, cout, hw, relu, w, grad_y, y_prev, gn_weight.contiguous(),
+                                             gn_bias.contiguous(), mean, rstd, gn_groups, grad_z, dsdb)
+            grad_prev, gw, gb = _gn_bwd_dx(nat, B, cin, hw, gn_groups, relu, y_prev, gn_weight, gn_bias, mean, rstd, grad_z, dsdb)
+            return grad_prev, None, gw, gb, grad_w.view_as(conv_weight), None, None, None, None, None, None
         if y_prev.dtype is torch.bfloat16 or (_gemm_ok(cout, hw) and _plain_gemm_mine(cout, (B, cin, hw))):
             grad_z = torch.empty_like(y_prev)
             nat.conv1x1_gemm_wrapper(B, cin, cout, hw, 1, w, grad_y, grad_z)
@@ -847,6 +868,14 @@
             grad_w = zeroed_empty((cout, cin), torch.float32, dev)
             nat.conv1x1_wgrad_affine_pooled_wrapper(B, cin, cout, hw, relu, S, y_prev, a, bb, y, coef2, inj, grad_w)
             grad_z = torch.empty_like(y_prev)
+            if (GN_SUMS_IN_DGRAD and y_prev.dtype is torch.float32 and y.dtype is torch.float32 and cin % gn_groups == 0
+                    and getattr(nat, "conv1x1_dgrad_pooled_gnsums_wrapper", None) is not None):
+                dsdb = zeroed_empty(2 * B * cin * nat.group_norm_bwd_slots(), torch.float64, dev)
+                nat.conv1x1_dgrad_pooled_gnsums_wrapper(B, cin, cout, hw, S, gn_groups, relu, w, y, coef2, inj, y_prev,
+                                                        gn_weight.contiguous(), gn_bias.contiguous(), mean, rstd, grad_z, dsdb)
+                grad_prev, gw, gb = _gn_bwd_dx(nat, B, cin, hw, gn_groups, relu, y_prev, gn_weight, gn_bias, mean, rstd, grad_z,
+                                               dsdb)
+                return (grad_prev, None, gw, gb, grad_w.view_as(conv_weight), None, None, None, gw2, gb2, None, None, None)
             nat.conv1x1_dgrad_pooled_wrapper(B, cin, cout, hw, S, w, y, coef2, inj, grad_z)
             grad_prev = torch.empty_like(y_prev)
             gw, gb = torch.empty_like(gn_weight), torch.empty_like(gn_bias)
diff --git a/ogc_amd/pointnet2_cuda.py b/ogc_amd/pointnet2_cuda.py
--- a/ogc_amd/pointnet2_cuda.py
+++ b/ogc_amd/pointnet2_cuda.py
@@ -404,6 +404,17 @@
          _f(grad_gamma, "grad_gamma"), _f(grad_beta, "grad_beta"), _check(ws, torch.float64, "ws"))
 
 
+def group_norm_bwd_slots():
+    return _lib.load().ogc_group_norm_bwd_slots()
+
+
+def group_norm_bwd_dx_wrapper(b, c, hw, groups, relu, x, gamma, beta, mean, rstd, grad_y, dsdb, slots, grad_x, grad_gamma,
+                              grad_beta):
+    _run("ogc_group_norm_bwd_dx", x, b, c, hw, groups, int(relu), _f(x, "x"), _f(gamma, "gamma"), _f(beta, "beta"),
+         _f(mean, "mean"), _f(rstd, "rstd"), _f(grad_y, "grad_y"), _check(dsdb, torch.float64, "dsdb"), int(slots),
+         _f(grad_x, "grad_x"), _f(grad_gamma, "grad_gamma"), _f(grad_beta, "grad_beta"))
+
+
 def group_norm_maxpool_fwd_wrapper(b, c, p, s, groups, eps, relu, x, gamma, beta, out, argmax, mean, rstd, ws):
     _run("ogc_group_norm_maxpool_fwd", x, b, c, p, s, groups, float(eps), int(relu), _f(x, "x"), _f(gamma, "gamma"),
          _f(beta, "beta"), _f(out, "out"), _i(argmax, "argmax"), _f(mean, "mean"), _f(rstd, "rstd"),
@@ -686,6 +697,23 @@
          yp, _f(coef2, "coef2"), _f(inj, "inj"), _f(dw, "dw"))
 
 
+def conv1x1_dgrad_pooled_gnsums_wrapper(b, cin, cout, hw, nsample, groups, relu, w, y, coef2, inj, y_prev, gamma, beta, mean,
+                                        rstd, grad_z, dsdb):
+    _run("ogc_conv1x1_dgrad_pooled_gnsums", y, b, cin, cout, hw, nsample, groups, int(relu), _f(w, "w"), _f(y, "y"),
+         _f(coef2, "coef2"), _f(inj, "inj"), _f(y_prev, "y_prev"), _f(gamma, "gamma"), _f(beta, "beta"), _f(mean, "mean"),
+         _f(rstd, "rstd"), _f(grad_z, "grad_z"), _check(dsdb, torch.float64, "dsdb"))
+
+
+def conv1x1_dgrad_gnsums_supported(b, cin, cout, hw):
+    return bool(_lib.load().ogc_conv1x1_dgrad_gnsums_supported(int(b), int(cin), int(cout), int(hw)))
+
+
+def conv1x1_dgrad_gnsums_wrapper(b, cin, cout, hw, relu, w, grad_y, y_prev, gamma, beta, mean, rstd, groups, grad_z, dsdb):
+    _run("ogc_conv1x1_dgrad_gnsums", grad_y, b, cin, cout, hw, int(relu), _f(w, "w"), _f(grad_y, "grad_y"), _f(y_prev, "y_prev"),
+         _f(gamma, "gamma"), _f(beta, "beta"), _f(mean, "mean"), _f(rstd, "rstd"), groups, _f(grad_z, "grad_z"),
+         _check(dsdb, torch.float64, "dsdb"))
+
+
 def conv1x1_dgrad_pooled_wrapper(b, cin, cout, hw, nsample, w, y, coef2, inj, grad_z):
     h, (yp, gp) = _acts((y, grad_z), ("y", "grad_z"))
     _run("ogc_conv1x1_dgrad_pooled" + h, y, b, cin, cout, hw, nsample, _f(w, "w"), yp, _f(coef2, "coef2"), _f(inj, "inj"), gp)
```

Result: no change. 1595 point-clouds/s, median of 3 (+1.7%).
